# radhofan/Fairify

Hardware: AMD Instinct MI355X
Metric: % partitions verified + partitions/sec on AC suite at 1/2/4/8 MI355X (higher is better)
Workload: dtype fp32

## Files before the change

### fairify_amd/csrc/bindings.cpp

```cpp
#include <hip/hip_runtime.h>
#include <pybind11/pybind11.h>
#include <pybind11/stl.h>

#include <algorithm>
#include <cmath>
#include <cstring>
#include <cstdint>
#include <stdexcept>
#include <vector>

#include "kwargs.h"
#include "runtime_host.h"

extern "C" int fa_bounds_launch(const NetDesc& net, BoundArgs args, hipStream_t stream);
extern "C" int fa_crown_phase_launch(const NetDesc& net, CrownPhaseArgs a, hipStream_t stream);
extern "C" size_t fa_crown_phase_bytes(const NetDesc& net);
extern "C" int fa_point_try_launch(const NetDesc& net, BoundArgs a, hipStream_t stream);
extern "C" int fa_forward_launch(const NetDesc& net, FwdArgs a, hipStream_t stream);
extern "C" int fa_sim_launch(const NetDesc& net, SimArgs a, hipStream_t stream);
extern "C" int fa_sim_shaped(const NetDesc& net);
extern "C" int fa_sym_shaped(const NetDesc& net, unsigned long long fold_mask);
extern "C" int fa_crown_shaped(const NetDesc& net, int mask);
extern "C" int fa_refine_shaped(const NetDesc& net, int logit);
extern "C" int fa_rate_launch(const NetDesc& net, RateArgs a, hipStream_t stream);
extern "C" int fa_count_enum_launch(const NetDesc& net, EnumArgs a, hipStream_t stream);
extern "C" int fa_count_rows_launch(CountArgs a, hipStream_t stream);
extern "C" int fa_count_level_launch(CountArgs a, hipStream_t stream);
extern "C" int fa_ascent_launch(const NetDesc& net, AscentArgs a, hipStream_t stream);
extern "C" int fa_certify_launch(CertArgs a, hipStream_t stream);
extern "C" int fa_falsify_launch(const NetDesc& net, FalsifyArgs a, hipStream_t stream);
extern "C" int fa_prune_masks_launch(const NetDesc& net, int P, const int* counts, const float* ub, int ub_stride,
                                     const uint8_t* sym_dead, uint8_t* code, int* cnt, hipStream_t stream);
extern "C" int fa_heuristic_launch(const NetDesc& net, int Pu, const int64_t* rows, const float* lb, const float* ub,
                                   int stride, const uint8_t* code, double q50, double qlo, double qhi, uint8_t* hnew,
                                   uint8_t* hmerged, int* hcnt, hipStream_t stream);
extern "C" int fa_agree_launch(const NetDesc& net, const float* flat, int Pm, const int64_t* rows, const float* lo,
                               const float* hi, const int64_t* pids, const uint8_t* dead, int S, uint32_t seed,
                               int* agree, hipStream_t stream);

extern "C" int fa_decode_launch(const DecodeDesc& d, const int64_t* ids, int P, const float* chunk_lo,
                                const float* chunk_hi, float* lo, float* hi, hipStream_t stream);
extern "C" int fa_trace_marker_launch(int tag, int* sink, hipStream_t stream);
extern "C" int fa_beta_launch(const NetDesc& nd, BetaArgs a, hipStream_t stream);
extern "C" int fa_beta_config(const NetDesc& nd, int* wpb, int* wtl, size_t* bytes);
extern "C" int fa_beta_opt16_fits(const NetDesc& nd);
extern "C" size_t fa_beta_opt16_scratch_floats(const NetDesc& nd, int R);
extern "C" int fa_beta_opt16_launch(const NetDesc& nd, BetaArgs a, float* pgsum, float* pgn, hipStream_t stream);
extern "C" int fa_beta_level16_launch(const NetDesc& nd, BetaArgs a, hipStream_t stream);
extern "C" int fa_beta_opt16_feas_launch(const NetDesc& nd, BetaArgs a, hipStream_t stream);
extern "C" int fa_beta_feas16_launch(const NetDesc& nd, BetaArgs a, hipStream_t stream);
extern "C" int fa_knn_launch(const float* X, int n, int d, int k, int* idx, float* dist, hipStream_t stream);
extern "C" int fa_actdiff_launch(const NetDesc& net, const float* flat, const float* x, const float* xp, int npairs,
                                 float* sum_out, hipStream_t stream);
extern "C" int fa_pack_masks_launch(const uint8_t* src, int P, int N, int stride, int sel, uint8_t* out, int NB,
                                    unsigned long long* hash, hipStream_t stream);

template <typename T>
static T* P(uintptr_t p) { return reinterpret_cast<T*>(p); }

using fa_rt::gamma_up;

struct Net {
  NetDesc d;
  explicit Net(const std::vector<int>& dims, double unit) {
    if (dims.size() < 2 || dims.size() > FA_MAX_LAYERS + 1) throw std::invalid_argument("bad layer count");
    std::memset(&d, 0, sizeof(d));
    d.n_layers = (int)dims.size() - 1;
    int off = 0, noff = 0, mw = 0, mws = 0;
    for (size_t i = 0; i < dims.size(); ++i) {
      d.dims[i] = dims[i];
      mw = std::max(mw, dims[i]);
    }
    for (int l = 0; l < d.n_layers; ++l) {
      d.w_off[l] = off;
      off += dims[l] * dims[l + 1];
      d.b_off[l] = off;
      off += dims[l + 1];
      d.neuron_off[l] = noff;
      noff += dims[l + 1];
      mws = std::max(mws, dims[l] * dims[l + 1]);
      d.g_gemm[l] = gamma_up(2 * dims[l] + 1, unit);
      d.g_fwd[l] = gamma_up(dims[l] + 1, unit);
    }
    d.n_neurons = noff;
    d.n_hidden = noff - dims.back();
    d.max_width = mw;
    d.max_wsize = mws;
    d.unit = (float)unit;
    d.g_conc = gamma_up(dims[0] + 1, unit);
    d.g_one = gamma_up(1, unit);
    n_params = off;
    d.wperm_off = (off + 3) & ~3;
    int wp = 0;
    for (int l = 0; l < d.n_layers; ++l) wp += ((dims[l] + 15) / 16) * ((dims[l + 1] + 15) / 16) * 256;
    for (int l = 0; l < d.n_layers; ++l) wp += dims[l + 1];
    d.wperm_floats = (wp + 3) & ~3;
    total_floats = d.wperm_off + d.wperm_floats;
    d.pack_g = 1;
    if (d.n_layers >= 2 && dims[0] <= 16 && mw <= 16) {
      int mh = 0;
      for (int l = 1; l < d.n_layers; ++l) mh = std::max(mh, dims[l]);
      d.pack_g = mh <= 4 ? 4 : (mh <= 8 ? 2 : 1);
    }
    d.pack_off = total_floats;
    d.pack_floats = 0;
    if (d.pack_g > 1) {
      d.pack_floats = d.pack_g * 256 + (d.n_layers - 1) * 256 + d.n_layers * 16;
      total_floats += d.pack_floats;
    }
    d.wback_off = total_floats;
    int wb = 0;
    for (int l = 0; l < d.n_layers; ++l) wb += ((dims[l] + 15) / 16) * ((dims[l + 1] + 15) / 16) * 256;
    d.wback_floats = wb;
    total_floats += wb;
  }
  int n_params;
  int total_floats;
};

const NetDesc& fa_net_desc(py::handle h) { return h.cast<const Net&>().d; }
void register_bab(py::module& m);
void register_relu(py::module& m);
void register_beta(py::module& m);
extern "C" int fa_crown_launch(const NetDesc& net, BoundArgs a, hipStream_t stream);
extern "C" int fa_refine_launch(const NetDesc& net, BoundArgs a, hipStream_t stream);
extern "C" int fa_backward_launch(const NetDesc& net, BoundArgs a, hipStream_t stream);
extern "C" int fa_refine_crown_launch(const NetDesc& net, BoundArgs a, hipStream_t stream);
void register_csv(py::module& m);

using fa_rt::ckl;

static hipStream_t finish(Kw& k) {
  const hipStream_t s = reinterpret_cast<hipStream_t>(k.u64("stream"));
  k.done();
  return s;
}

static int dims(Kw& k, const char* key, int* idx, size_t cap, const char* too_many) {
  const std::vector<int> v = k.ints(key);
  if (v.size() > cap) throw std::invalid_argument(too_many);
  std::copy(v.begin(), v.end(), idx);
  return (int)v.size();
}

enum { OUT = 1, FORMS = 2, LAYERS = 4 };
template <typename A>
static A row_args(Kw& k, int req, const char* lo = "lo", const char* hi = "hi") {
  auto p = [&](const char* key, int group) { return (req & group) ? k.need<float>(key) : k.ptr<float>(key); };
  A a{};
  a.flat = k.need<const float>("flat");
  a.lo = k.need<const float>(lo);
  a.hi = k.need<const float>(hi);
  a.R = k.i("R");
  a.out_lb = p("out_lb", OUT);
  a.out_ub = p("out_ub", OUT);
  a.Lc = p("Lc", FORMS); a.L0 = p("L0", FORMS); a.Le = p("Le", FORMS);
  a.Uc = p("Uc", FORMS); a.U0 = p("U0", FORMS); a.Ue = p("Ue", FORMS);
  a.layer_lb = p("layer_lb", LAYERS);
  a.layer_ub = p("layer_ub", LAYERS);
  return a;
}
static BoundArgs bound_args(Kw& k, int req, const char* lo = "lo", const char* hi = "hi") {
  BoundArgs a = row_args<BoundArgs>(k, req, lo, hi);
  a.dead_in = k.ptr<const uint8_t>("dead_in");
  return a;
}

template <typename A>
static void fill_query(A& a, Kw& k, const char* too_many) {
  a.flat = k.need<const float>("flat");
  a.lo = k.need<const float>("lo");
  a.hi = k.need<const float>("hi");
  a.P = k.i("P");
  a.V = k.i("V");
  a.npa = dims(k, "pa", a.pa_idx, FA_MAX_PA, too_many);
  a.values = k.ptr<const int64_t>("values");
  a.Pp = k.i("Pp");
  a.pairs = k.ptr<const int64_t>("pairs");
}
template <typename A>
static void fill_samples(A& a, Kw& k, const char* too_many) {
  a.pids = k.need<const int64_t>("pids");
  a.n_samples = k.i("n_samples");
  a.seed = (uint32_t)k.u64("seed");
  a.nra = dims(k, "ra", a.ra_idx, FA_MAX_RA, too_many);
  a.tau = k.i("tau");
}
template <typename A>
static void fill_ascent(A& a, Kw& k, const char* too_many) {
  a.K = k.i("K");
  a.iters = k.i("iters");
  a.nfree = dims(k, "free", a.free_idx, 64, too_many);
  a.found = k.need<uint8_t>("found");
  a.wit_x = k.need<float>("wit_x");
  a.wit_xp = k.need<float>("wit_xp");
}

static BetaArgs beta_args(const Net& net, Kw& k) {
  BetaArgs a;
  std::memset(&a, 0, sizeof(a));
  a.flat = k.need<const float>("flat");
  a.wt = k.ptr<const float>("wt");
  a.R = k.i("R");
  a.npa = dims(k, "pa", a.pa_idx, FA_MAX_PA, "beta_level: too many PA dims");
  for (int q = 0; q < a.npa; ++q)
    if (a.pa_idx[q] < 0 || a.pa_idx[q] >= net.d.dims[0] || (q && a.pa_idx[q] <= a.pa_idx[q - 1]))
      throw std::invalid_argument("beta_level: PA dims must be increasing input indices");
  a.lo = k.need<const float>("lo");
  a.hi = k.need<const float>("hi");
  a.va = k.need<const float>("va");
  a.vb = k.need<const float>("vb");
  a.LBA = k.need<const float>("LBA");
  a.UBA = k.need<const float>("UBA");
  a.LBB = k.need<const float>("LBB");
  a.UBB = k.need<const float>("UBB");
  a.phA = k.need<const int8_t>("phA");
  a.phB = k.need<const int8_t>("phB");
  a.par = k.need<float>("par");
  a.t = k.need<float>("t");
  a.scratch = k.need<float>("scratch");
  a.iters = k.i("iters");
  a.lr_a = k.f("lr_a");
  a.lr_b = k.f("lr_b");
  a.lr_t = k.f("lr_t");
  a.decay = k.f("decay");
  a.lookahead = k.i("lookahead", 0);
  a.beta_pos = k.i("beta_pos", 1);
  const int flags = k.i("flags", 0);
  a.stall = flags & 1;
  a.pgap = (flags >> 1) & 3;
  a.feas = (flags >> 3) & 1;
  a.bound = k.ptr<double>("bound");
  a.split = k.ptr<int>("split");
  a.xstar = k.ptr<float>("xstar");
  a.binit = k.ptr<float>("binit");
  a.ramask = k.u64("ramask", 0);
  a.plo = k.ptr<const float>("plo");
  a.phi = k.ptr<const float>("phi");
  a.xpstar = k.ptr<float>("xpstar");
  a.gtie = k.ptr<float>("gtie");
  a.tau = k.f("tau", 0.f);
  a.osg = k.ptr<const int8_t>("osg");
  a.pgsum = k.ptr<const float>("pgsum");
  a.pgn = k.ptr<const float>("pgn");
  a.fpar = k.ptr<float>("fpar");
  a.fgt = k.ptr<float>("fgt");
  a.fval = k.ptr<double>("fval");
  if ((net.d.dims[0] < 64 && (a.ramask >> net.d.dims[0])) || (a.ramask && (!a.plo || !a.phi)))
    throw std::invalid_argument("beta_level: RA mask beyond the inputs or no x' box");
  return a;
}

PYBIND11_MODULE(_C, m) {
  m.doc() = "fairify_amd CDNA4 (gfx950) kernels";
  py::class_<Net>(m, "Net")
      .def(py::init<const std::vector<int>&, double>())
      .def_readonly("n_params", &Net::n_params)
      .def_readonly("total_floats", &Net::total_floats)
      .def_property_readonly("wperm_off", [](const Net& n) { return n.d.wperm_off; })
      .def_property_readonly("pack_g", [](const Net& n) { return n.d.pack_g; })
      .def_property_readonly("pack_off", [](const Net& n) { return n.d.pack_off; })
      .def_property_readonly("n_hidden", [](const Net& n) { return n.d.n_hidden; })
      .def_property_readonly("n_neurons", [](const Net& n) { return n.d.n_neurons; });

  m.def("bounds", [](const Net& net, py::kwargs kw) {
    Kw k("bounds", kw);
    const int symbolic = k.i("symbolic");
    BoundArgs a = bound_args(k, symbolic ? OUT | FORMS : OUT);
    a.symbolic = symbolic;
    a.G = k.i("G", 0);
    a.dead_out = k.ptr<uint8_t>("dead_out");
    a.fold = k.u64("fold", 0);
    a.phase_in = k.ptr<const int8_t>("phase_in");
    a.infeas = k.ptr<uint8_t>("infeas");
    ckl(fa_bounds_launch(net.d, a, finish(k)), "bounds");
  });

  m.def("crown_phase", [](const Net& net, py::kwargs kw) {
    Kw k("crown_phase", kw);
    CrownPhaseArgs a = row_args<CrownPhaseArgs>(k, OUT | FORMS | LAYERS);
    a.phase = k.ptr<const int8_t>("phase");
    a.infeas = k.ptr<const uint8_t>("infeas");
    a.split = k.need<int>("split");
    a.score = k.need<float>("score");
    a.low = k.ptr<float>("low");
    const int rc = fa_crown_phase_launch(net.d, a, finish(k));
    if (rc != 0) throw std::runtime_error("crown_phase launch failed, code " + std::to_string(rc));
  });

  m.def("relu_fits", [](const Net& net) { return fa_crown_phase_bytes(net.d) > 0; });

  m.def("crown", [](const Net& net, py::kwargs kw) {
    Kw k("crown", kw);
    const BoundArgs a = bound_args(k, OUT | FORMS | LAYERS);
    ckl(fa_crown_launch(net.d, a, finish(k)), "crown");
  });

  m.def("refine", [](const Net& net, py::kwargs kw) {
    Kw k("refine", kw);
    BoundArgs a = bound_args(k, LAYERS);
    a.phase_in = k.ptr<const int8_t>("phase_in");
    a.infeas = k.ptr<uint8_t>("infeas");
    const int rc = fa_refine_launch(net.d, a, finish(k));
    if (rc < -1) throw std::runtime_error("refine launch failed, code " + std::to_string(rc));
    return rc;
  });
  m.def("refine_crown", [](const Net& net, py::kwargs kw) {
    Kw k("refine_crown", kw);
    const BoundArgs a = bound_args(k, OUT | FORMS | LAYERS);
    const int rc = fa_refine_crown_launch(net.d, a, finish(k));
    if (rc < -1) throw std::runtime_error("refine_crown launch failed, code " + std::to_string(rc));
    return rc;
  });
  m.def("backward_bounds", [](const Net& net, py::kwargs kw) {
    Kw k("backward_bounds", kw);
    const BoundArgs a = bound_args(k, OUT | FORMS);
    const int rc = fa_backward_launch(net.d, a, finish(k));
    if (rc < -1) throw std::runtime_error("backward_bounds launch failed, code " + std::to_string(rc));
    return rc;
  });

  m.def("point_bounds", [](const Net& net, py::kwargs kw) {
    Kw k("point_bounds", kw);
    BoundArgs a = bound_args(k, OUT, "x", "x");
    a.row_open = k.ptr<const uint8_t>("row_open");
    a.open_mod = k.i("open_mod", 0);
    if (a.row_open && a.open_mod <= 0) throw std::invalid_argument("point_bounds: row_open needs open_mod > 0");
    const hipStream_t stream = finish(k);
    const int rc = fa_point_try_launch(net.d, a, stream);
    if (rc < 0) ckl(-rc, "point_bounds");
    if (rc == 0) ckl(fa_bounds_launch(net.d, a, stream), "point_bounds(ibp)");
  });

  m.def("forward", [](const Net& net, uintptr_t flat, uintptr_t x, int B, uintptr_t dead, uintptr_t out,
                      uintptr_t stream) {
    FwdArgs a{};
    a.flat = P<const float>(flat);
    a.x = P<const float>(x);
    a.B = B;
    a.dead = P<const uint8_t>(dead);
    a.out = P<float>(out);
    ckl(fa_forward_launch(net.d, a, (hipStream_t)stream), "forward");
  });

  m.def("sim", [](const Net& net, py::kwargs kw) {
    Kw k("sim", kw);
    SimArgs a{};
    fill_query(a, k, "too many PA/RA dims");
    fill_samples(a, k, "too many PA/RA dims");
    a.counts = k.need<int>("counts");
    a.found = k.need<uint8_t>("found");
    a.wit_x = k.need<float>("wit_x");
    a.wit_xp = k.need<float>("wit_xp");
    a.z0 = k.ptr<float>("z0");
    a.keys = k.ptr<int>("keys");
    a.split = k.i("split");
    a.regcount = k.i("regcount");
    if (a.split < 1 || (a.split > 1 && !a.keys)) throw std::invalid_argument("sim: split > 1 needs a keys buffer");
    ckl(fa_sim_launch(net.d, a, finish(k)), "sim");
  });
  m.def("sim_shaped", [](const Net& net) { return fa_sim_shaped(net.d) != 0; });
  m.def("sym_shaped", [](const Net& net, unsigned long long fold) { return fa_sym_shaped(net.d, fold) != 0; });
  m.def("crown_shaped", [](const Net& net, bool mask) { return fa_crown_shaped(net.d, mask) != 0; });
  m.def("refine_shaped", [](const Net& net, bool logit) { return fa_refine_shaped(net.d, logit) != 0; });

  m.def("rate", [](const Net& net, py::kwargs kw) {
    Kw k("rate", kw);
    RateArgs a{};
    fill_query(a, k, "too many PA/RA dims");
    fill_samples(a, k, "too many PA/RA dims");
    a.E = k.i("E");
    a.flips = k.need<int>("flips");
    a.amb = k.need<int>("amb");
    a.amb_idx = k.need<int>("amb_idx");
    a.split = k.i("split");
    const int rc = fa_rate_launch(net.d, a, finish(k));
    if (rc == -3) throw std::invalid_argument("rate: shape not covered (layer > 160, inputs > 32, V > 32 or E > 32)");
    ckl(rc, "rate");
  });

  m.def("count_enum", [](const Net& net, py::kwargs kw) {
    Kw k("count_enum", kw);
    EnumArgs a{};
    a.flat = k.need<const float>("flat");
    a.lo = k.need<const float>("lo");
    a.hi = k.need<const float>("hi");
    a.L = k.i("L");
    a.V = k.i("V");
    a.npa = dims(k, "pa", a.pa_idx, FA_MAX_PA, "too many PA/RA dims");
    a.values = k.need<const int64_t>("values");
    a.Pp = k.i("Pp");
    a.pairs = k.ptr<const int64_t>("pairs");
    a.nra = dims(k, "ra", a.ra_idx, FA_MAX_RA, "too many PA/RA dims");
    a.tau = k.i("tau");
    a.E = k.i("E");
    a.max_vol = k.i("max_vol");
    a.cert = k.need<int>("cert");
    a.amb = k.need<int>("amb");
    a.amb_idx = k.need<int>("amb_idx");
    a.blocks = k.i("blocks");
    if (a.Pp > 0 && !a.pairs) throw py::type_error("count_enum() missing required keyword argument 'pairs'");
    const int rc = fa_count_enum_launch(net.d, a, finish(k));
    if (rc == -3)
      throw std::invalid_argument(
          "count_enum: shape not covered (layer > 160, inputs > 32, V > 32, E > 32 or leaf volume > 65536)");
    ckl(rc, "count_enum");
  });
  auto count_args = [](Kw& k) {
    CountArgs a{};
    a.N = k.i("N");
    a.n0 = k.i("n0");
    a.V = k.i("V");
    a.npa = dims(k, "pa", a.pa_idx, FA_MAX_PA, "too many PA/RA dims");
    a.lo = k.need<const float>("lo");
    a.hi = k.need<const float>("hi");
    return a;
  };
  m.def("count_rows", [count_args](py::kwargs kw) {
    Kw k("count_rows", kw);
    CountArgs a = count_args(k);
    a.nra = dims(k, "ra", a.ra_idx, FA_MAX_RA, "too many PA/RA dims");
    a.tau = k.f("tau");
    a.values = k.need<const float>("values");
    a.rlo = k.need<float>("rlo");
    a.rhi = k.need<float>("rhi");
    a.plo = k.ptr<float>("plo");
    a.phi = k.ptr<float>("phi");
    ckl(fa_count_rows_launch(a, finish(k)), "count_rows");
  });
  m.def("count_level", [count_args](py::kwargs kw) {
    Kw k("count_level", kw);
    CountArgs a = count_args(k);
    a.part = k.need<const int>("part");
    a.lx = k.need<const float>("lx");
    a.ux = k.need<const float>("ux");
    a.lxp = k.need<const float>("lxp");
    a.uxp = k.need<const float>("uxp");
    a.Pp = k.i("Pp");
    a.pairs = k.ptr<const int64_t>("pairs");
    a.score = k.need<const float>("score");
    a.leaf_points = (long long)k.u64("leaf_points");
    a.code = k.need<uint8_t>("code");
    a.fair = k.need<long long>("fair");
    a.unfair = k.need<long long>("unfair");
    a.child_cnt = k.need<int>("child_cnt");
    a.olo = k.need<float>("olo");
    a.ohi = k.need<float>("ohi");
    a.opart = k.need<int>("opart");
    a.cap = k.i("cap");
    a.leaf_lo = k.need<float>("leaf_lo");
    a.leaf_hi = k.need<float>("leaf_hi");
    a.leaf_part = k.need<int>("leaf_part");
    a.leaf_cap = k.i("leaf_cap");
    a.counters = k.need<int>("counters");
    if (a.Pp > 0 && !a.pairs) throw py::type_error("count_level() missing required keyword argument 'pairs'");
    ckl(fa_count_level_launch(a, finish(k)), "count_level");
  });

  m.def("ascent", [](const Net& net, py::kwargs kw) {
    Kw k("ascent", kw);
    AscentArgs a{};
    fill_query(a, k, "too many PA/free dims");
    fill_ascent(a, k, "too many PA/free dims");
    a.x0 = k.need<const float>("x0");
    a.f0 = k.need<const float>("f0");
    a.q0 = k.need<const int>("q0");
    const int rc = fa_ascent_launch(net.d, a, finish(k));
    if (rc == -1) return false;
    ckl(rc, "ascent");
    return true;
  });

  m.def("falsify", [](const Net& net, py::kwargs kw) {
    Kw k("falsify", kw);
    FalsifyArgs a{};
    fill_query(a, k, "too many PA/RA/free dims");
    fill_samples(a, k, "too many PA/RA/free dims");
    fill_ascent(a, k, "too many PA/RA/free dims");
    if (a.tau <= 0) {
      a.nra = 0;
      std::fill_n(a.ra_idx, FA_MAX_RA, 0);
    }
    a.n_local = k.i("n_local");
    a.walk_k = k.i("walk_k");
    a.walk_steps = k.i("walk_steps");
    a.how = k.need<int8_t>("how");
    a.dseed = (uint32_t)k.u64("dseed");
    const int rc = fa_falsify_launch(net.d, a, finish(k));
    if (rc == 0) return false;
    if (rc < 0) ckl(-rc, "falsify");
    return true;
  });


  m.def("prune_masks", [](const Net& net, int Pn, uintptr_t counts, uintptr_t ub, int ub_stride, uintptr_t sym_dead,
                          uintptr_t code, uintptr_t cnt, uintptr_t stream) {
    ckl(fa_prune_masks_launch(net.d, Pn, P<const int>(counts), P<const float>(ub), ub_stride,
                                P<const uint8_t>(sym_dead), P<uint8_t>(code), P<int>(cnt), (hipStream_t)stream),
          "prune_masks");
  });

  m.def("heuristic", [](const Net& net, int Pu, uintptr_t rows, uintptr_t lb, uintptr_t ub, int stride, uintptr_t code,
                        double q50, double qlo, double qhi, uintptr_t hnew, uintptr_t hmerged, uintptr_t hcnt,
                        uintptr_t stream) {
    ckl(fa_heuristic_launch(net.d, Pu, P<const int64_t>(rows), P<const float>(lb), P<const float>(ub), stride,
                              P<const uint8_t>(code), q50, qlo, qhi, P<uint8_t>(hnew), P<uint8_t>(hmerged),
                              P<int>(hcnt), (hipStream_t)stream),
          "heuristic");
  });

  m.def("agree", [](const Net& net, uintptr_t flat, int Pm, uintptr_t rows, uintptr_t lo, uintptr_t hi, uintptr_t pids,
                    uintptr_t dead, int S, uint32_t seed, uintptr_t agree, uintptr_t stream) {
    const int rc = fa_agree_launch(net.d, P<const float>(flat), Pm, P<const int64_t>(rows), P<const float>(lo),
                                   P<const float>(hi), P<const int64_t>(pids), P<const uint8_t>(dead), S, seed,
                                   P<int>(agree), (hipStream_t)stream);
    if (rc == 0) return false;
    if (rc < 0) ckl(-rc, "agree");
    return true;
  });

  m.def("certify", [](py::kwargs kw) {
    Kw k("certify", kw);
    auto in = [&](const char* key) { return k.need<const float>(key); };
    CertArgs a{};
    a.Nn = k.i("Nn"); a.n0 = k.i("n0"); a.V = k.i("V"); a.Pp = k.i("Pp"); a.norient = k.i("norient");
    a.Lc = in("Lc"); a.L0 = in("L0"); a.Le = in("Le"); a.Uc = in("Uc"); a.U0 = in("U0"); a.Ue = in("Ue");
    a.olb = in("olb"); a.oub = in("oub");
    a.Lcp = in("Lcp"); a.L0p = in("L0p"); a.Lep = in("Lep"); a.Ucp = in("Ucp"); a.U0p = in("U0p"); a.Uep = in("Uep");
    a.olbp = in("olbp"); a.oubp = in("oubp");
    a.xlo = in("xlo"); a.xhi = in("xhi"); a.xplo = in("xplo"); a.xphi = in("xphi");
    a.pairs = k.ptr<const int64_t>("pairs");
    a.values = k.ptr<const int64_t>("values");
    a.npa = dims(k, "pa", a.pa_idx, FA_CMAX_PA, "too many PA/RA dims");
    a.nra = dims(k, "ra", a.ra_idx, FA_MAX_RA, "too many PA/RA dims");
    a.tau = k.f("tau");
    a.shared = k.need<const uint8_t>("shared");
    a.unit = k.f("unit");
    a.gmarg = std::nextafter(k.f("gmarg"), INFINITY);
    a.gmin = k.ptr<float>("gmin"); a.tstar = k.ptr<float>("tstar");
    a.open = k.need<uint8_t>("open"); a.score = k.need<float>("score"); a.split_dim = k.need<int64_t>("split_dim");
    a.cand_x = k.need<float>("cand_x"); a.cand_xp = k.need<float>("cand_xp");
    a.cand_v = k.need<int64_t>("cand_v"); a.cand_o = k.need<int64_t>("cand_o");
    a.scores = k.ptr<float>("scores"); a.leaf = k.ptr<uint8_t>("leaf");
    a.skip_closed = k.i("skip_closed", 0);
    a.status = k.ptr<const int8_t>("status"); a.part = k.ptr<const int>("part");
    a.smear = k.i("smear", 0);
    a.lay_lb = k.ptr<const float>("lay_lb"); a.lay_ub = k.ptr<const float>("lay_ub"); a.lay_N = k.i("lay_N", 0);
    a.W0T = k.ptr<const float>("W0T"); a.n1 = k.i("n1", 0);
    if ((a.status == nullptr) != (a.part == nullptr)) throw std::invalid_argument("certify: status and part go together");
    if (a.smear && (!a.lay_lb || !a.lay_ub || !a.W0T || a.n1 <= 0 || a.lay_N < a.n1))
      throw std::invalid_argument("certify: smear needs lay_lb, lay_ub, W0T and 0 < n1 <= lay_N");
    ckl(fa_certify_launch(a, finish(k)), "certify");
  });

  m.def("decode", [](std::vector<int> radix, std::vector<long long> div, std::vector<int> chunk_off,
                     std::vector<float> base_lo, std::vector<float> base_hi, uintptr_t ids, int Pn,
                     uintptr_t chunk_lo, uintptr_t chunk_hi, uintptr_t lo, uintptr_t hi, uintptr_t stream) {
    const size_t n0 = radix.size();
    if (n0 == 0 || n0 > FA_DECODE_MAX_DIMS || div.size() != n0 || chunk_off.size() != n0 || base_lo.size() != n0 ||
        base_hi.size() != n0)
      throw std::invalid_argument("decode: descriptor sizes");
    DecodeDesc d{};
    d.n0 = (int)n0;
    for (size_t k = 0; k < n0; ++k) {
      if (radix[k] < 0 || (radix[k] > 0 && div[k] <= 0)) throw std::invalid_argument("decode: radix/div");
      d.radix[k] = radix[k];
      d.div[k] = div[k];
      d.chunk_off[k] = chunk_off[k];
      d.base_lo[k] = base_lo[k];
      d.base_hi[k] = base_hi[k];
    }
    ckl(fa_decode_launch(d, P<const int64_t>(ids), Pn, P<const float>(chunk_lo), P<const float>(chunk_hi),
                           P<float>(lo), P<float>(hi), (hipStream_t)stream),
          "decode");
  });
  m.def("pack_masks", [](uintptr_t src, int Pn, int N, int stride, int sel, uintptr_t out, int NB, uintptr_t hash,
                         uintptr_t stream) {
    ckl(fa_pack_masks_launch(P<const uint8_t>(src), Pn, N, stride, sel, P<uint8_t>(out), NB,
                               P<unsigned long long>(hash), (hipStream_t)stream),
          "pack_masks");
  });
  m.def("knn", [](uintptr_t X, int n, int d, int k, uintptr_t idx, uintptr_t dist, uintptr_t stream) {
    ckl(fa_knn_launch(P<const float>(X), n, d, k, P<int>(idx), P<float>(dist), (hipStream_t)stream), "knn");
  });
  m.def("actdiff", [](const Net& net, uintptr_t flat, uintptr_t x, uintptr_t xp, int npairs, uintptr_t sum_out,
                      uintptr_t stream) {
    ckl(fa_actdiff_launch(net.d, P<const float>(flat), P<const float>(x), P<const float>(xp), npairs,
                            P<float>(sum_out), (hipStream_t)stream),
          "actdiff");
  });
  m.def("trace_marker", [](int tag, uintptr_t sink, uintptr_t stream) {
    ckl(fa_trace_marker_launch(tag, P<int>(sink), (hipStream_t)stream), "trace_marker");
  });
  m.def("beta_level", [](const Net& net, py::kwargs kw) {
    Kw k("beta_level", kw);
    const BetaArgs a = beta_args(net, k);
    return fa_beta_launch(net.d, a, finish(k));
  });
  m.def("beta_level16", [](const Net& net, py::kwargs kw) {
    Kw k("beta_level16", kw);
    const BetaArgs a = beta_args(net, k);
    return fa_beta_level16_launch(net.d, a, finish(k));
  });
  m.def("beta_opt16", [](const Net& net, py::kwargs kw) {
    Kw k("beta_opt16", kw);
    BetaArgs a = beta_args(net, k);
    float* pgsum = const_cast<float*>(a.pgsum);
    float* pgn = const_cast<float*>(a.pgn);
    a.wt = a.pgsum = a.pgn = nullptr;
    return fa_beta_opt16_launch(net.d, a, pgsum, pgn, finish(k));
  });
  m.def("beta_feas", [](const Net& net, py::kwargs kw) {
    Kw k("beta_feas", kw);
    BetaArgs a = beta_args(net, k);
    const int mode = k.i("mode");
    const hipStream_t st = finish(k);
    if (mode < 0 || mode > 3) throw std::invalid_argument("beta_feas: mode must be 0..3");
    if (mode != 0 && !a.fpar) throw std::invalid_argument("beta_feas: fpar required");
    a.lookahead = a.stall = a.pgap = 0;
    a.beta_pos = a.feas = 1;
    a.split = nullptr;
    a.xstar = a.binit = a.xpstar = nullptr;
    if (mode == 0) {
      a.fpar = a.fgt = nullptr;
      return fa_beta_launch(net.d, a, st);
    }
    if (mode == 1) return fa_beta_feas16_launch(net.d, a, st);
    if (mode == 2) return fa_beta_opt16_feas_launch(net.d, a, st);
    a.iters = 0;
    return fa_beta_launch(net.d, a, st);
  });
  m.def("beta_batched_fits", [](const Net& net) { return fa_beta_opt16_fits(net.d) != 0; });
  m.def("beta_opt16_scratch", [](const Net& net, int R) { return fa_beta_opt16_scratch_floats(net.d, R); });
  m.def("beta_config", [](const Net& net) {
    int w = 0, t = 0;
    size_t b = 0;
    const int rc = fa_beta_config(net.d, &w, &t, &b);
    return py::make_tuple(rc, w, t, b);
  });
  m.def("beta_fits", [](const Net& net) {
    int w = 0, t = 0;
    size_t b = 0;
    return fa_beta_config(net.d, &w, &t, &b) == 0;
  });
  m.def("arch", []() { return std::string("gfx950"); });
  m.def("prepare_lds", [] { return fa_lds_prepare(); });
  m.def("lds_registered", [] { return (int)fa_lds_registry().size(); });
  register_bab(m);
  register_relu(m);
  register_beta(m);
  m.def("mem_stats", [] {
    const fa_mem::Stats s = fa_mem::stats();
    py::dict d;
    d["dev_cached_bytes"] = s.dev_cached_bytes;
    d["dev_live_bytes"] = s.dev_live_bytes;
    d["host_cached_bytes"] = s.host_cached_bytes;
    d["host_live_bytes"] = s.host_live_bytes;
    d["dev_mallocs"] = s.dev_mallocs;
    d["dev_hits"] = s.dev_hits;
    d["host_mallocs"] = s.host_mallocs;
    d["host_hits"] = s.host_hits;
    d["driver_frees"] = s.driver_frees;
    return d;
  });
  m.def("mem_release_cached", [] { fa_mem::release_cached(); });
  register_csv(m);
}
```

### fairify_amd/csrc/symbolic.hip

```cpp
#include <hip/hip_runtime.h>

#include <tuple>

#include "args.h"
#include "launch.h"

#define FA_SYM_MAXC 48

struct SymCfg {
  int nc;
  int cdim[FA_SYM_MAXC];
  unsigned long long fold;
  int w_lds[FA_MAX_LAYERS];
  int b_lds[FA_MAX_LAYERS];
  int lds_floats;
  int stage_off;
  int stage_floats;
};

using SymShapeAny = FaShapeAny;
template <int... D>
using SymShape = FaShape<D...>;

struct SymBox {
  const BoundArgs* a;
  int node, v, n0;
  __device__ __forceinline__ float lo(int d) const {
    float x = a->lo[(size_t)node * n0 + d];
    if (a->V > 0)
      for (int k = 0; k < a->npa; ++k)
        if (a->pa_idx[k] == d) x = a->values[v * a->npa + k];
    return x;
  }
  __device__ __forceinline__ float hi(int d) const {
    float x = a->hi[(size_t)node * n0 + d];
    if (a->V > 0)
      for (int k = 0; k < a->npa; ++k)
        if (a->pa_idx[k] == d) x = a->values[v * a->npa + k];
    return x;
  }
};

__device__ __forceinline__ int fa_trot(int rho) { return rho >> 3; }

template <int NT, int PG = 1>
struct SymSlab {
  static constexpr int TS = 16 * NT + 4;
  static constexpr int TILE1 = 2 * 16 * TS;
  static constexpr int TILE = 2 * TILE1;
  static constexpr int BOX = 3 * FA_SYM_MAXC;
  static constexpr int BOXTAB = PG > 1 ? 2 * PG * 32 : 0;
  static constexpr int FLOATS = (TILE + 2 * PG * BOX + BOXTAB + 3) & ~3;
};

template <bool PAIR, int TM>
struct SymForm {
  static constexpr bool CR = !PAIR && TM >= 2;
};

__device__ __forceinline__ void fa_pq_to_ul(const f32x4& P, const f32x4& Q, int fc, float gg, f32x4& U,
                                            f32x4& L) {
  const float sl = (fc == 1 || fc == 3) ? 2.f * gg : 0.f;
#pragma unroll
  for (int i = 0; i < 4; ++i) {
    const float q = Q[i], e = sl * fabsf(q);
    U[i] = (P[i] + q) + e;
    L[i] = (P[i] - q) - e;
  }
}

template <int NT, bool PAIR, int PG = 1, bool CR = false, class S = SymShapeAny>
__device__ __forceinline__ bool fa_sym_epilogue(const NetDesc& net, const BoundArgs& a, const SymCfg& cfg,
                                                const float* smem, float* T, const float* bxv_in, const int* cdim_s,
                                                int l, int r_in, int node_in, int r2, int node2, bool v2, int lane,
                                                int jt0, const f32x4 (&U)[2][NT],
                                                const f32x4 (&Lq)[2][NT], float (&nu)[2][NT][4],
                                                float (&nlo)[2][NT][4]) {
  constexpr int TS = SymSlab<NT>::TS;
  constexpr bool CS = S::L > 0;
  const int col = lane & 15, grp = lane >> 4;
  const int n_out = CS ? S::dim(l + 1) : net.dims[l + 1];
  const float* sb = smem + cfg.b_lds[l];
  const bool last = CS ? l == S::L - 1 : l == net.n_layers - 1;
  const float gg = net.g_gemm[l];
  const float gc = net.g_conc;
  const float gi = net.g_one;
  const float unit = net.unit;
  const float gnext = last ? 0.f : (CR ? net.g_fwd[l + 1] : net.g_gemm[l + 1]);
  const int noff = net.neuron_off[l];
  const int nc = cfg.nc;
  const int n0 = CS ? S::dim(0) : net.dims[0];
  const int tsub = lane >> 5;
  const bool second = PAIR && tsub;
  constexpr int PS = 16 / PG;
  const int gbox = PG > 1 ? col / PS : 0;
  const int bidx = tsub * PG + gbox;
  const int r = PG > 1 ? r_in + bidx : (second ? r2 : r_in);
  const int node = PG > 1 ? (a.V > 0 ? r / a.V : r) : (second ? node2 : node_in);
  const float* bxv = bxv_in + (PG > 1 ? bidx : (second ? 1 : 0)) * SymSlab<NT, PG>::BOX;
  const int jt = PAIR ? jt0 : jt0 + tsub;
  const int n_out_t = n_out;
  const bool nl_act = PG > 1 ? r < a.R : (16 * jt < n_out_t && (!second || v2));
  const int ob = (lane >> 4) & 1;
  float* Trow = T + tsub * SymSlab<NT>::TILE1 + (ob * 16 + col) * TS + fa_trot(ob * 16 + col);
#pragma unroll
    for (int u = 0; u < 2; ++u)
#pragma unroll
      for (int ct = 0; ct < NT; ++ct)
#pragma unroll
        for (int i = 0; i < 4; ++i) {
          const int ru = 4 * grp + i, rl = 16 + 4 * grp + i;
          T[u * SymSlab<NT>::TILE1 + ru * TS + fa_trot(ru) + ct * 16 + col] = U[u][ct][i];
          T[u * SymSlab<NT>::TILE1 + rl * TS + fa_trot(rl) + ct * 16 + col] = Lq[u][ct][i];
        }
    __builtin_amdgcn_wave_barrier();
    const int j = PG > 1 ? col - gbox * PS : 16 * jt + col;
    const bool jv = j < n_out;
    float v[16 * NT];
#pragma unroll
    for (int c = 0; c < 16 * NT; ++c) v[c] = Trow[c];
    const float braw = sb[PG > 1 ? col : min(j, n_out - 1)];
    const float b = jv ? braw : 0.f;
    float s1 = 0.f, s2 = 0.f, mg = 0.f;
#pragma unroll
    for (int c = 4; c < 16 * NT; ++c) {
      const float av = fabsf(v[c]);
      s1 = fmaf(v[c], bxv[c], s1);
      s2 = fmaf(av, bxv[FA_SYM_MAXC + c], s2);
      mg = fmaf(av, bxv[2 * FA_SYM_MAXC + c], mg);
    }
    float mn = s1 - s2, mx = s1 + s2;
    const float cr = v[0];
    float er = v[1], ivr = v[2], ier = v[3];
    const float sgn = ob ? -1.f : 1.f;
    er *= sgn;
    ier *= sgn;
    const float c0 = cr + b;
    const float mgc = mg;
    mn += c0; mx += c0; mg += fabsf(c0);
    const float iv = ivr + b;
    const float eI = ier * (1.f + 2.f * gg) + gg * fabsf(b);
    const float e = er * (1.f + 2.f * gg) + gg * fabsf(b);
    float bound;
    if (ob == 0) bound = fminf(iv + gi * fabsf(iv) + eI, mx + gc * mg + e);
    else bound = fmaxf(iv - gi * fabsf(iv) - eI, mn - gc * mg - e);
    const float other = __shfl_xor(bound, 16, 64);
    const float ub = ob == 0 ? bound : other;
    const float lb = ob == 0 ? other : bound;
    if (nl_act && jv && a.layer_lb) {
      if (ob == 0) a.layer_ub[(size_t)r * net.n_neurons + noff + j] = ub;
      else a.layer_lb[(size_t)r * net.n_neurons + noff + j] = lb;
    }
    if (last) {
      if (nl_act && j == 0) {
        float* Cf = ob == 0 ? a.Uc : a.Lc;
        if (ob == 0) {
          a.out_ub[r] = ub; a.U0[r] = c0; a.Ue[r] = e;
        } else {
          a.out_lb[r] = lb; a.L0[r] = c0; a.Le[r] = e;
        }
        for (int d = 0; d < n0; ++d)
          if ((cfg.fold >> d) & 1ull) Cf[(size_t)r * n0 + d] = 0.f;
        for (int c = 0; c < nc; ++c) Cf[(size_t)r * n0 + cdim_s[c]] = Trow[4 + c];
      }
      return false;
    }
    bool forced = false, fact = false;
    if (nl_act && jv) {
      if (a.dead_in) forced = a.dead_in[(size_t)r * net.n_hidden + noff + j] != 0;
      else if (a.dead_part) forced = a.dead_part[(size_t)a.node_part[node] * net.n_hidden + noff + j] != 0;
      if (a.phase_in) {
        const int8_t ph = a.phase_in[(size_t)r * net.n_hidden + noff + j];
        forced = forced || ph < 0;
        fact = ph > 0;
        if (ob == 0 && a.infeas && ((ph < 0 && lb > 0.f) || (ph > 0 && ub < 0.f))) a.infeas[r] = 1;
      }
    }
    const bool isdead = ub <= 0.f;
    const bool isact = lb >= 0.f;
    if (nl_act && ob == 0 && jv && a.dead_out) a.dead_out[(size_t)r * net.n_hidden + noff + j] = isdead ? 1 : 0;
    const bool zero = isdead || forced || !jv;
    const float aa = mn - gc * mg + e;
    const float bb = mx + gc * mg + e;
    const bool chord = !zero && !isact && !fact && aa < 0.f;
    const float sc = (bb / (bb - aa)) * (1.f + 4.f * unit);
    const float shift = e - aa;
    const float cc = c0 * sc + sc * shift;
    const float sU = zero ? 0.f : (chord ? sc : 1.f);
    const float cU = zero ? 0.f : (chord ? cc : c0);
    const float mU = zero ? 0.f : (chord ? sc * mgc * (1.f + 8.f * unit) + fabsf(cc) : mg);
    const float eU = zero ? 0.f : (chord ? 4.f * unit * sc * (mg + fabsf(shift)) : e);
    const float aL = mn - gc * mg - e;
    const float bL = mx + gc * mg - e;
    const bool lam1 = !zero && (isact || ((bL > 0.f) && (bL > -aL)));
    const bool up = ob == 0;
    const float ivn = zero ? 0.f : fmaxf(up ? ub : lb, 0.f);
    const float s = up ? sU : (lam1 ? 1.f : 0.f);
    const float cnew = up ? cU : (lam1 ? c0 : 0.f);
    const float en = up ? eU : (lam1 ? e : 0.f);
    const float mgn = up ? mU : (lam1 ? mg : 0.f);
    const float mg_b = CR ? mgn + __shfl_xor(mgn, 16, 64) : mgn;
    const float iv_b = CR ? fmaxf(ivn, __shfl_xor(ivn, 16, 64)) : ivn;
    v[0] = cnew;
    v[1] = sgn * (en + gnext * mg_b);
    v[2] = ivn;
    v[3] = sgn * (gnext * iv_b);
#pragma unroll
    for (int c = 4; c < 16 * NT; ++c) v[c] *= s;
    if (nl_act) {
#pragma unroll
      for (int c = 0; c < 16 * NT; ++c) Trow[c] = v[c];
    }
    __builtin_amdgcn_wave_barrier();
#pragma unroll
    for (int u = 0; u < 2; ++u)
#pragma unroll
      for (int ct = 0; ct < NT; ++ct)
#pragma unroll
        for (int i = 0; i < 4; ++i) {
          const int ru = 4 * grp + i, rl = 16 + 4 * grp + i;
          const float xu = T[u * SymSlab<NT>::TILE1 + ru * TS + fa_trot(ru) + ct * 16 + col];
          const float xl = T[u * SymSlab<NT>::TILE1 + rl * TS + fa_trot(rl) + ct * 16 + col];
          nu[u][ct][i] = CR ? 0.5f * (xu + xl) : xu;
          nlo[u][ct][i] = CR ? 0.5f * (xu - xl) : xl;
        }
    __builtin_amdgcn_wave_barrier();
    return true;
}

template <int NT, int TM, bool PAIR, int PG = 1, class S = SymShapeAny>
__device__ __forceinline__ void fa_sym_layer(const NetDesc& net, const BoundArgs& a, const SymCfg& cfg,
                                             const float* smem, float* T, const float* bxv, const int* cdim_s,
                                             int l, int r, int node, int r2, int node2, bool v2, int lane,
                                             const float (&B)[NT][PAIR ? 2 : TM][2][4],
                                             float (&A)[NT][PAIR ? 2 : TM][2][4]) {
  constexpr int TMS = PAIR ? 2 : TM;
  constexpr bool CR = SymForm<PAIR, TM>::CR;
  constexpr int TS = SymSlab<NT>::TS;
  constexpr bool CS = S::L > 0;
  const int col = lane & 15, grp = lane >> 4;
  const int n_in = CS ? S::dim(l) : net.dims[l], n_out = CS ? S::dim(l + 1) : net.dims[l + 1];
  const int tin = (n_in + 15) >> 4, tout = (n_out + 15) >> 4;
  const float* sw = smem + cfg.w_lds[l];
  const float* sb = smem + cfg.b_lds[l];
  const bool last = CS ? l == S::L - 1 : l == net.n_layers - 1;
  const float gg = net.g_gemm[l];
  const float gc = net.g_conc;
  const float gi = net.g_one;
  const float unit = net.unit;
  const float gnext = last ? 0.f : net.g_gemm[l + 1];
  const int noff = net.neuron_off[l];
  const int nc = cfg.nc;
  const int n0 = CS ? S::dim(0) : net.dims[0];
  const bool nl_act = lane < 32;
  const int ob = (lane >> 4) & 1;
#ifndef FA_SYM_TIMING_NO_EPILOGUE
  if (PG > 1 && l == 0) {
    const float* boxtab = bxv + 2 * PG * SymSlab<NT, PG>::BOX;
    const float g0 = net.g_gemm[0];
    const int n0v = n0;
    f32x4 U[2][NT], Lq[2][NT];
#pragma unroll
    for (int u = 0; u < 2; ++u) {
#pragma unroll
      for (int ct = 0; ct < NT; ++ct) U[u][ct] = Lq[u][ct] = f32x4{0.f, 0.f, 0.f, 0.f};
#pragma unroll
      for (int g = 0; g < PG; ++g) {
        const float* bt = boxtab + (u * PG + g) * 32;
        const float4 w4 = reinterpret_cast<const float4*>(sw)[g * 64 + lane];
        const float wv[4] = {w4.x, w4.y, w4.z, w4.w};
#pragma unroll
        for (int i = 0; i < 4; ++i) {
          const int k = 4 * grp + i;
          const bool kv = k < n0v;
          const float xl = kv ? bt[k] : 0.f, xh = kv ? bt[16 + k] : 0.f;
          const bool folded = kv && ((cfg.fold >> k) & 1ull);
          const float m = fmaxf(fabsf(xl), fabsf(xh));
          const float wp = fmaxf(wv[i], 0.f), wn = fminf(wv[i], 0.f);
#pragma unroll
          for (int ct = 0; ct < NT; ++ct) {
            const int c = ct * 16 + col;
            float vu = 0.f, vl = 0.f;
            if (kv) {
              if (c >= 4) {
                vu = vl = (!folded && c - 4 < nc && cdim_s[c - 4] == k) ? 1.f : 0.f;
              } else if (c == 0) {
                vu = vl = folded ? xl : 0.f;
              } else if (c == 1) {
                vu = g0 * m; vl = -vu;
              } else if (c == 2) {
                vu = xh; vl = xl;
              } else {
                vu = g0 * fabsf(xh); vl = -(g0 * fabsf(xl));
              }
            }
            U[u][ct] = fa_mfma4(wp, vu, U[u][ct]);
            Lq[u][ct] = fa_mfma4(wp, vl, Lq[u][ct]);
            U[u][ct] = fa_mfma4(wn, vl, U[u][ct]);
            Lq[u][ct] = fa_mfma4(wn, vu, Lq[u][ct]);
          }
        }
      }
    }
    float nu[2][NT][4], nlo[2][NT][4];
    if (!fa_sym_epilogue<NT, PAIR, PG, CR, S>(net, a, cfg, smem, T, bxv, cdim_s, l, r, node, r2, node2, v2, lane, 0, U, Lq,
                                       nu, nlo))
      return;
#pragma unroll
    for (int u = 0; u < 2; ++u)
#pragma unroll
      for (int ct = 0; ct < NT; ++ct)
#pragma unroll
        for (int i = 0; i < 4; ++i) {
          A[ct][u][0][i] = nu[u][ct][i];
          A[ct][u][1][i] = nlo[u][ct][i];
        }
    return;
  }
  if (PG == 1 && last && n_out == 1) {
    constexpr int NB = PAIR ? 2 : 1;
    float su[NB][NT], sl[NB][NT];
#pragma unroll
    for (int bi = 0; bi < NB; ++bi)
#pragma unroll
      for (int ct = 0; ct < NT; ++ct) su[bi][ct] = sl[bi][ct] = 0.f;
#pragma unroll
    for (int t = 0; t < TM; ++t) {
      if (t >= tin) break;
      const float4 w4 = reinterpret_cast<const float4*>(sw)[t * 64 + grp * 16];
      const float wv[4] = {w4.x, w4.y, w4.z, w4.w};
#pragma unroll
      for (int i = 0; i < 4; ++i) {
        const float wp = fmaxf(wv[i], 0.f), wn = fminf(wv[i], 0.f);
#pragma unroll
        for (int bi = 0; bi < NB; ++bi)
#pragma unroll
          for (int ct = 0; ct < NT; ++ct) {
            const int bt = PAIR ? bi : t;
            if (CR) {
              su[bi][ct] = fmaf(wv[i], B[ct][bt][0][i], su[bi][ct]);
              sl[bi][ct] = fmaf(fabsf(wv[i]), B[ct][bt][1][i], sl[bi][ct]);
            } else {
              su[bi][ct] = fmaf(wp, B[ct][bt][0][i], fmaf(wn, B[ct][bt][1][i], su[bi][ct]));
              sl[bi][ct] = fmaf(wp, B[ct][bt][1][i], fmaf(wn, B[ct][bt][0][i], sl[bi][ct]));
            }
          }
      }
    }
    f32x4 U[2][NT], Lq[2][NT];
#pragma unroll
    for (int ct = 0; ct < NT; ++ct) U[1][ct] = Lq[1][ct] = f32x4{0.f, 0.f, 0.f, 0.f};
#pragma unroll
    for (int bi = 0; bi < NB; ++bi)
#pragma unroll
      for (int ct = 0; ct < NT; ++ct) {
        float xu = su[bi][ct], xl = sl[bi][ct];
        xu += __shfl_xor(xu, 16, 64);
        xl += __shfl_xor(xl, 16, 64);
        xu += __shfl_xor(xu, 32, 64);
        xl += __shfl_xor(xl, 32, 64);
        U[bi][ct] = f32x4{grp == 0 ? xu : 0.f, 0.f, 0.f, 0.f};
        Lq[bi][ct] = f32x4{grp == 0 ? xl : 0.f, 0.f, 0.f, 0.f};
        if (CR) fa_pq_to_ul(f32x4(U[bi][ct]), f32x4(Lq[bi][ct]), ct * 16 + col, gg, U[bi][ct], Lq[bi][ct]);
      }
    float nu[2][NT][4], nlo[2][NT][4];
    fa_sym_epilogue<NT, PAIR, PG, CR, S>(net, a, cfg, smem, T, bxv, cdim_s, l, r, node, r2, node2, v2, lane, 0, U, Lq,
                                  nu, nlo);
    return;
  }
#endif
#pragma unroll
  for (int jt0 = 0; jt0 < TM; jt0 += 2) {
    if (jt0 >= tout) break;
    f32x4 U[2][NT], Lq[2][NT];
#pragma unroll
    for (int u = 0; u < 2; ++u) {
      const int jt = jt0 + u;
#pragma unroll
      for (int ct = 0; ct < NT; ++ct) {
        U[u][ct] = f32x4{0.f, 0.f, 0.f, 0.f};
        Lq[u][ct] = f32x4{0.f, 0.f, 0.f, 0.f};
      }
      if (PAIR ? (jt0 > 0) : (jt >= tout || jt >= TM)) continue;
      const float4* wq = reinterpret_cast<const float4*>(sw) + (size_t)(PAIR ? 0 : jt) * tin * 64 + lane;
#pragma unroll
      for (int t = 0; t < TM; ++t) {
        if (t >= tin) break;
        const float4 w4 = wq[t * 64];
        const float wv[4] = {w4.x, w4.y, w4.z, w4.w};
#pragma unroll
        for (int i = 0; i < 4; ++i) {
          const float wp = fmaxf(wv[i], 0.f), wn = fminf(wv[i], 0.f);
#pragma unroll
          for (int ct = 0; ct < NT; ++ct) {
            const int bt = PAIR ? u : t;
            const float bu = B[ct][bt][0][i], bl = B[ct][bt][1][i];
            if (CR) {
              U[u][ct] = fa_mfma4(wv[i], bu, U[u][ct]);
              Lq[u][ct] = fa_mfma4(fabsf(wv[i]), bl, Lq[u][ct]);
            } else {
              U[u][ct] = fa_mfma4(wp, bu, U[u][ct]);
              Lq[u][ct] = fa_mfma4(wp, bl, Lq[u][ct]);
              U[u][ct] = fa_mfma4(wn, bl, U[u][ct]);
              Lq[u][ct] = fa_mfma4(wn, bu, Lq[u][ct]);
            }
          }
        }
      }
      if (CR) {
#pragma unroll
        for (int ct = 0; ct < NT; ++ct)
          fa_pq_to_ul(f32x4(U[u][ct]), f32x4(Lq[u][ct]), ct * 16 + col, gg, U[u][ct], Lq[u][ct]);
      }
    }
    float nu[2][NT][4], nlo[2][NT][4];
#ifdef FA_SYM_TIMING_NO_EPILOGUE
#pragma unroll
    for (int u = 0; u < 2; ++u)
#pragma unroll
      for (int ct = 0; ct < NT; ++ct)
#pragma unroll
        for (int i = 0; i < 4; ++i) {
          nu[u][ct][i] = U[u][ct][i] * 1e-3f;
          nlo[u][ct][i] = Lq[u][ct][i] * 1e-3f;
        }
    if (l == net.n_layers - 1) {
      if (lane == 0) a.out_lb[r] = nu[0][0][0] + nlo[0][0][1];
      continue;
    }
#else
    if (!fa_sym_epilogue<NT, PAIR, PG, CR, S>(net, a, cfg, smem, T, bxv, cdim_s, l, r, node, r2, node2, v2, lane, jt0, U,
                                       Lq, nu, nlo))
      continue;
#endif
#pragma unroll
    for (int u = 0; u < 2; ++u) {
      if (jt0 + u >= TMS) break;
#pragma unroll
      for (int ct = 0; ct < NT; ++ct)
#pragma unroll
        for (int i = 0; i < 4; ++i) {
          A[ct][jt0 + u][0][i] = nu[u][ct][i];
          A[ct][jt0 + u][1][i] = nlo[u][ct][i];
        }
    }
  }
}

#ifndef FA_SYM_WPE7
#define FA_SYM_WPE7 2
#endif
#ifndef FA_SYM_WPE4
#define FA_SYM_WPE4 2
#endif
#define FA_SYM_WAVES_PER_EU(NT, TM, PAIR) \
  ((PAIR) ? 3 : ((TM) == 2 ? 3 : ((TM) == 4 ? FA_SYM_WPE4 : ((TM) == 7 ? FA_SYM_WPE7 : 1))))

template <int NT, int TM, bool PAIR, int PG, class S, int... LS>
__device__ __forceinline__ void fa_sym_layers_c(std::integer_sequence<int, LS...>, const NetDesc& net,
                                                const BoundArgs& a, const SymCfg& cfg, const float* smem, float* T,
                                                const float* bxv, const int* cdim_s, int r, int node, int r2,
                                                int node2, bool v2, int lane, float (&XA)[NT][PAIR ? 2 : TM][2][4],
                                                float (&XB)[NT][PAIR ? 2 : TM][2][4]) {
  ((LS & 1 ? fa_sym_layer<NT, TM, PAIR, PG, S>(net, a, cfg, smem, T, bxv, cdim_s, LS, r, node, r2, node2, v2, lane,
                                               XB, XA)
           : fa_sym_layer<NT, TM, PAIR, PG, S>(net, a, cfg, smem, T, bxv, cdim_s, LS, r, node, r2, node2, v2, lane,
                                               XA, XB)),
   ...);
}

#ifndef FA_SYM_BIG_THREADS
#define FA_SYM_BIG_THREADS 512
#endif
#define FA_SYM_THREADS(TM) ((TM) == 7 ? FA_SYM_BIG_THREADS : FA_THREADS)

template <int NT, int TM, bool PAIR, int PG = 1, class S = SymShapeAny>
__global__ void __launch_bounds__(FA_SYM_THREADS(TM)) __attribute__((amdgpu_waves_per_eu(FA_SYM_WAVES_PER_EU(NT, TM, PAIR))))
fa_sym_kernel(NetDesc net, BoundArgs a, SymCfg cfg) {
  constexpr bool CR = SymForm<PAIR, TM>::CR;
  constexpr int TMS = PAIR ? 2 : TM;
  extern __shared__ __attribute__((aligned(16))) float smem[];
  const int tid = threadIdx.x;
  {
    const float4* src = reinterpret_cast<const float4*>(a.flat + cfg.stage_off);
    float4* dst = reinterpret_cast<float4*>(smem);
    for (int e = tid; e < (cfg.stage_floats >> 2); e += FA_SYM_THREADS(TM)) dst[e] = src[e];
  }
  int* cdim_s = reinterpret_cast<int*>(smem + cfg.lds_floats - FA_SYM_MAXC);
  for (int c = tid; c < FA_SYM_MAXC; c += FA_SYM_THREADS(TM)) cdim_s[c] = c < cfg.nc ? cfg.cdim[c] : -1;
  __syncthreads();
  const int lane = tid & 63;
  const int grp = lane >> 4;
  const int wave = tid >> 6;
  const int nw = FA_SYM_THREADS(TM) / 64;
  const int n0 = S::L > 0 ? S::dim(0) : net.dims[0];
  const int nc = cfg.nc;
  const float g0 = net.g_gemm[0];
  float* T = smem + cfg.lds_floats + wave * SymSlab<NT, PG>::FLOATS;
  float* bxv = T + SymSlab<NT>::TILE;
  const int tin0 = (n0 + 15) >> 4;
  int role[NT], cdm[NT];
#pragma unroll
  for (int ct = 0; ct < NT; ++ct) {
    const int c = ct * 16 + (lane & 15);
    role[ct] = c == 0 ? 1 : c == 1 ? 2 : c == 2 ? 3 : c == 3 ? 4 : (c - 4 < nc ? 0 : 5);
    cdm[ct] = (role[ct] == 0) ? cdim_s[c - 4] : -1;
  }
  constexpr int RPW = PAIR ? 2 * PG : 1;
  for (int r0 = (blockIdx.x * nw + wave) * RPW; r0 < a.R; r0 += gridDim.x * nw * RPW) {
    const int r = __builtin_amdgcn_readfirstlane(r0);
    const bool v2 = PAIR && r + 1 < a.R;
    const int rb = v2 ? r + 1 : r;
    if (a.skip_status) {
      bool any = false;
#pragma unroll
      for (int bi = 0; bi < RPW; ++bi) {
        const int rr = min(r + bi, a.R - 1);
        const int8_t s1 = a.skip_status[a.skip_part[a.V > 0 ? rr / a.V : rr]];
        any = any || s1 == 3 || s1 == 4;
      }
      if (!any) continue;
    }
    SymBox bxs[RPW];
#pragma unroll
    for (int bi = 0; bi < RPW; ++bi) {
      SymBox& bx = bxs[bi];
      const int rr = PG > 1 ? min(r + bi, a.R - 1) : (bi ? rb : r);
      bx.a = &a;
      bx.n0 = n0;
      bx.node = a.V > 0 ? rr / a.V : rr;
      bx.v = a.V > 0 ? rr - bx.node * a.V : 0;
      if (lane < FA_SYM_MAXC) {
        float* bv = bxv + bi * SymSlab<NT>::BOX;
        const int d = (lane >= 4 && lane - 4 < nc) ? cdim_s[lane - 4] : -1;
        const float l0 = d >= 0 ? bx.lo(d) : 0.f, h0 = d >= 0 ? bx.hi(d) : 0.f;
        float mid = 0.5f * (l0 + h0), rad = 0.5f * (h0 - l0), mm = fmaxf(fabsf(l0), fabsf(h0));
        const bool lattice = l0 == rintf(l0) && h0 == rintf(h0) && fabsf(l0) < 4194304.f && fabsf(h0) < 4194304.f;
        if (!lattice) {
          rad = nextafterf(fmaxf(h0 - mid, mid - l0), INFINITY);
          mm = nextafterf(fabsf(mid) + rad, INFINITY);
        }
        bv[lane] = mid;
        bv[FA_SYM_MAXC + lane] = rad;
        bv[2 * FA_SYM_MAXC + lane] = mm;
      }
      if (PG > 1 && lane < 32) {
        const int d = lane & 15;
        float* bt = bxv + 2 * PG * SymSlab<NT, PG>::BOX + bi * 32;
        bt[lane] = d < n0 ? (lane < 16 ? bx.lo(d) : bx.hi(d)) : 0.f;
      }
    }
    const SymBox& bx = bxs[0];
    float XA[NT][TMS][2][4], XB[NT][TMS][2][4];
#pragma unroll
    for (int t = 0; t < TMS; ++t) {
      if (PG > 1) break;
      if (!PAIR && t >= tin0) break;
      const SymBox& bt = bxs[PAIR ? t : 0];
#pragma unroll
      for (int i = 0; i < 4; ++i) {
        const int k = (PAIR ? 0 : 16 * t) + 4 * grp + i;
        float xl = 0.f, xh = 0.f;
        const bool kv = k < n0;
        if (kv) {
          xl = bt.lo(k);
          xh = bt.hi(k);
        }
        const bool folded = kv && ((cfg.fold >> k) & 1ull);
        const float m = fmaxf(fabsf(xl), fabsf(xh));
#pragma unroll
        for (int ct = 0; ct < NT; ++ct) {
          float vu = 0.f, vl = 0.f;
          if (kv) {
            switch (role[ct]) {
              case 0: vu = (!folded && cdm[ct] == k) ? 1.f : 0.f; vl = CR ? 0.f : vu; break;
              case 1: vu = folded ? xl : 0.f; vl = CR ? 0.f : vu; break;
              case 2: vu = CR ? 0.f : g0 * m; vl = CR ? g0 * m : -vu; break;
              case 3:
                vu = CR ? 0.5f * (xh + xl) : xh;
                vl = CR ? 0.5f * (xh - xl) : xl;
                break;
              case 4:
                vu = CR ? 0.5f * g0 * (fabsf(xh) - fabsf(xl)) : g0 * fabsf(xh);
                vl = CR ? 0.5f * g0 * (fabsf(xh) + fabsf(xl)) : -(g0 * fabsf(xl));
                break;
              default: break;
            }
          }
          XA[ct][t][0][i] = vu;
          XA[ct][t][1][i] = vl;
        }
      }
    }
    __builtin_amdgcn_wave_barrier();
    if constexpr (S::L > 0) {
      fa_sym_layers_c<NT, TM, PAIR, PG, S>(std::make_integer_sequence<int, S::L>{}, net, a, cfg, smem, T, bxv, cdim_s,
                                           r, bx.node, rb, bxs[RPW - 1].node, v2, lane, XA, XB);
    } else {
      for (int l = 0; l < net.n_layers; ++l) {
        if (l & 1)
          fa_sym_layer<NT, TM, PAIR, PG>(net, a, cfg, smem, T, bxv, cdim_s, l, r, bx.node, rb, bxs[RPW - 1].node, v2,
                                         lane, XB, XA);
        else
          fa_sym_layer<NT, TM, PAIR, PG>(net, a, cfg, smem, T, bxv, cdim_s, l, r, bx.node, rb, bxs[RPW - 1].node, v2,
                                         lane, XA, XB);
      }
    }
    __builtin_amdgcn_wave_barrier();
  }
}


namespace {

typedef void (*SymKernel)(NetDesc, BoundArgs, SymCfg);

template <int NT, int TM, bool PAIR = false, int PG = 1>
SymKernel sym_ptr() {
  return fa_sym_kernel<NT, TM, PAIR, PG>;
}

bool use_pack() {
  static const bool v = [] {
    const char* e = getenv("FAIRIFY_SYM_PACK");
    return !(e && *e == '0');
  }();
  return v;
}

SymKernel select_packed(int pg) {
  switch (pg) {
    case 2: return sym_ptr<1, 1, true, 2>();
    case 4: return sym_ptr<1, 1, true, 4>();
    default: return nullptr;
  }
}

bool use_pair() {
  static const bool v = [] {
    const char* e = getenv("FAIRIFY_SYM_PAIR");
    return !(e && *e == '0');
  }();
  return v;
}

int max_tm() {
  static const int v = [] {
    const char* e = getenv("FAIRIFY_SYM_MAX_TM");
    return (e && *e) ? atoi(e) : 10;
  }();
  return v;
}

#define FA_SYM_GRID(X) X(1, 1) X(1, 2) X(1, 4) X(1, 7) X(1, 10) X(2, 1) X(2, 2) X(2, 4) X(2, 10) X(3, 1) X(3, 2)

int tm_bucket(int NT, int TM) {
  if (TM > max_tm()) return 0;
  const int b = fa_tm_bucket(TM);
  if (NT == 2 && b == 7) return 10;
  if (NT == 3 && b > 2) return 0;
  return NT >= 1 && NT <= 3 ? b : 0;
}

SymKernel select_kernel(int NT, int tmb) {
  if (NT == 1 && tmb == 1 && use_pair()) return sym_ptr<1, 1, true>();
  switch (16 * NT + tmb) {
#define FA_SYM_CASE(NT_, TM_) \
  case 16 * NT_ + TM_: return sym_ptr<NT_, TM_>();
    FA_SYM_GRID(FA_SYM_CASE)
#undef FA_SYM_CASE
    default: return nullptr;
  }
}

#define FA_SYM_SHAPES(X)                                                                              \
  X(1, 4, false, 1, 13, 64, 32, 16, 8, 4, 1)                \
  X(2, 4, false, 1, 13, 64, 32, 16, 8, 4, 1)          \
  X(2, 4, false, 1, 16, 64, 32, 16, 8, 4, 1)                                                \
  X(1, 4, false, 1, 13, 64, 64, 1)                                                          \
  X(1, 4, false, 1, 13, 50, 1)                                                              \
  X(1, 7, false, 1, 13, 100, 100, 1)                                                        \
  X(1, 7, false, 1, 13, 100, 1)                                                             \
               \
  X(1, 1, true, 1, 13, 16, 8, 1)                                                            \
  X(1, 1, true, 1, 13, 12, 12, 1)                                                           \
  X(1, 1, true, 1, 13, 10, 10, 10, 10, 1)                                                  \
                                                         \
  X(1, 1, true, 2, 13, 5, 5, 1)                                                             \
  X(1, 1, true, 2, 13, 5, 5, 5, 5, 1)

constexpr int sym_key(int nt, int tm, bool pair, int pg) { return ((16 * nt + tm) * 2 + (pair ? 1 : 0)) * 8 + pg; }

struct SymPick {
  SymKernel k;
  int NT, tmb;
  bool pair;
  int pg;
  bool shaped;
};

SymPick pick_sym(const NetDesc& net, unsigned long long fold_mask, SymCfg& cfg) {
  SymPick p{};
  const int n0 = net.dims[0];
  if (n0 > 64) return p;
  cfg.fold = fold_mask;
  int nc = 0;
  for (int d = 0; d < n0; ++d)
    if (!((fold_mask >> d) & 1ull)) {
      if (nc >= FA_SYM_MAXC) return p;
      cfg.cdim[nc++] = d;
    }
  cfg.nc = nc;
  const int cols = nc + 4;
  p.NT = (cols + 15) / 16;
  p.tmb = tm_bucket(p.NT, fa_widest_tiles(net, 0, net.n_layers));
  SymKernel k = select_kernel(p.NT, p.tmb);
  if (!k) return p;
  p.pair = k == sym_ptr<1, 1, true>();
  p.pg = (p.pair && net.pack_g > 1 && net.dims[0] <= 16 && use_pack()) ? net.pack_g : 1;
  if (p.pg > 1) k = select_packed(p.pg);
  if (!k) return p;
  if (!fa_env_off("FAIRIFY_SYM_SHAPED")) {
#define FA_SYM_ENTRY(NT, TM, PAIR, PG, ...) \
  {sym_key(NT, TM, PAIR, PG), {__VA_ARGS__}, fa_sym_kernel<NT, TM, PAIR, PG, SymShape<__VA_ARGS__>>},
    static const std::vector<FaShaped<SymKernel>> v = {FA_SYM_SHAPES(FA_SYM_ENTRY)};
#undef FA_SYM_ENTRY
    if (const SymKernel ks = fa_find_shaped(v, net, sym_key(p.NT, p.tmb, p.pair, p.pg))) {
      k = ks;
      p.shaped = true;
    }
  }
  p.k = k;
  return p;
}

}

extern "C" int fa_sym_shaped(const NetDesc& net, unsigned long long fold_mask) {
  SymCfg cfg{};
  return pick_sym(net, fold_mask, cfg).shaped;
}

extern "C" int fa_sym_try_launch(const NetDesc& net, BoundArgs a, unsigned long long fold_mask,
                                 hipStream_t stream) {
  if (!a.symbolic || a.R <= 0) return 0;
  SymCfg cfg{};
  const SymPick p = pick_sym(net, fold_mask, cfg);
  const SymKernel k = p.k;
  if (!k) return 0;
  const int NT = p.NT, tmb = p.tmb, pg = p.pg;
  const bool pair0 = p.pair;
  int off = 0;
  if (pg > 1) {
    cfg.w_lds[0] = 0;
    off = pg * 256;
    for (int l = 1; l < net.n_layers; ++l) {
      cfg.w_lds[l] = off;
      off += 256;
    }
    for (int l = 0; l < net.n_layers; ++l) {
      cfg.b_lds[l] = off;
      off += 16;
    }
    if (off != net.pack_floats) return -1;
    cfg.stage_off = net.pack_off;
  } else {
    off = fa_lay_weights(net, net.n_layers, cfg.w_lds, 0);
    off = fa_lay_biases(net, net.n_layers, cfg.b_lds, off);
    off = ((off + 3) & ~3);
    if (off != net.wperm_floats) return -1;
    cfg.stage_off = net.wperm_off;
  }
  cfg.stage_floats = off;
  off += FA_SYM_MAXC;
  cfg.lds_floats = off;
  int slab = 0;
  switch (NT) {
    case 1:
      slab = pg == 2 ? SymSlab<1, 2>::FLOATS : pg == 4 ? SymSlab<1, 4>::FLOATS : SymSlab<1>::FLOATS;
      break;
    case 2: slab = SymSlab<2>::FLOATS; break;
    default: slab = SymSlab<3>::FLOATS; break;
  }
  const int threads = (!pair0 && NT == 1 && tmb == 7) ? FA_SYM_BIG_THREADS : FA_THREADS;
  const int rows_per_block = (threads / 64) * (pair0 ? 2 * pg : 1);
  const size_t bytes = (size_t)(off + (threads / 64) * slab) * sizeof(float);
  if (bytes > 160 * 1024) return 0;
  const int per_cu = fa_blocks_per_cu((const void*)k, threads, bytes);
  if (!per_cu) return -4;
  long long blocks = (a.R + rows_per_block - 1) / rows_per_block;
  const long long cap = (long long)fa_device_cus() * per_cu;
  if (blocks > cap) blocks = cap;
  hipLaunchKernelGGL(k, dim3((unsigned)blocks), dim3(threads), bytes, stream, net, a, cfg);
  const hipError_t e = hipGetLastError();
  return e == hipSuccess ? 1 : -(int)e;
}

#define FA_SYM_LDS(NT, TM) FA_LDS_K((sym_ptr<NT, TM>())),
#define FA_SYM_SHAPE_LDS(NT, TM, PAIR, PG, ...) FA_LDS_K((fa_sym_kernel<NT, TM, PAIR, PG, SymShape<__VA_ARGS__>>)),
FA_LDS_REGISTER(FA_SYM_GRID(FA_SYM_LDS) FA_LDS_K((sym_ptr<1, 1, true>())), FA_LDS_K((sym_ptr<1, 1, true, 2>())),
                FA_LDS_K((sym_ptr<1, 1, true, 4>())));
FA_LDS_REGISTER(FA_SYM_SHAPES(FA_SYM_SHAPE_LDS));
#undef FA_SYM_LDS
#undef FA_SYM_SHAPE_LDS
```

### fairify_amd/ops/hip.py

```python
from __future__ import annotations

import os
import threading
from typing import Optional, Sequence

import torch

from . import ext
from . import reference as ref


def _stream(dev) -> int:
    return torch.cuda.current_stream(dev).cuda_stream


_LAZY_LOCK = threading.Lock()


def _net(be):
    n = getattr(be, "_hipnet", None)
    if n is None:
        with _LAZY_LOCK:
            n = getattr(be, "_hipnet", None)
            if n is None:
                dims = [be.mlp.n_in] + be.mlp.widths
                n = ext().Net(dims, be.unit)
                assert n.total_floats == be.flat.numel(), (n.total_floats, be.flat.numel())
                be._hipnet = n
    return n


def _c(t: torch.Tensor, dtype, shape=None, name="tensor") -> torch.Tensor:
    if t.dtype != dtype:
        t = t.to(dtype)
    t = t.contiguous()
    if shape is not None and tuple(t.shape) != tuple(shape):
        raise ValueError(f"{name}: expected shape {tuple(shape)}, got {tuple(t.shape)}")
    return t


def _fold_mask(fold: Sequence[int], n0: int) -> int:
    m = 0
    for d in fold:
        if not 0 <= int(d) < min(n0, 64):
            raise ValueError(f"fold dim {d} out of range")
        m |= 1 << int(d)
    return m


def _ptr(t: Optional[torch.Tensor]) -> int:
    return 0 if t is None else t.data_ptr()


def _ptrs(**tensors) -> dict:
    return {k: t.data_ptr() for k, t in tensors.items() if t is not None}


def _bound_kw(be, lo, hi, dead=None, res=None, layer_lb=None, layer_ub=None):
    R, n0 = lo.shape
    t = dict(flat=be.flat, lo=_c(lo, torch.float32, (R, n0), "lo"), hi=_c(hi, torch.float32, (R, n0), "hi"),
             dead_in=None if dead is None else _c(dead, torch.uint8, (R, be.n_hidden), "dead"),
             layer_lb=layer_lb, layer_ub=layer_ub)
    if res is not None:
        t.update(out_lb=res.out_lb, out_ub=res.out_ub, Lc=res.Lc, L0=res.L0, Le=res.Le, Uc=res.Uc, U0=res.U0,
                 Ue=res.Ue)
    return dict(_ptrs(**t), R=R, stream=_stream(lo.device)), t


def _layer_views(be, lay_lb, lay_ub):
    offs = [0]
    for w in be.mlp.widths:
        offs.append(offs[-1] + w)
    n = len(be.mlp.widths)
    return [lay_lb[:, offs[i]:offs[i + 1]] for i in range(n)], [lay_ub[:, offs[i]:offs[i + 1]] for i in range(n)]


def decode(grid, ids: torch.Tensor):
    dev = ids.device
    ids = _c(ids, torch.int64, (ids.shape[0],), "ids")
    tabs = grid.__dict__.setdefault("_dev_decode", {})
    key = str(dev)
    if key not in tabs:
        with _LAZY_LOCK:
            if key not in tabs:
                d = grid.decode_desc()
                cl = torch.from_numpy(d["chunk_lo"]).to(dev) if d["chunk_lo"].size else torch.zeros(1, device=dev)
                ch = torch.from_numpy(d["chunk_hi"]).to(dev) if d["chunk_hi"].size else torch.zeros(1, device=dev)
                torch.cuda.current_stream(dev).synchronize()
                tabs[key] = (d, cl, ch)
    d, cl, ch = tabs[key]
    n0 = int(d["radix"].shape[0])
    Pn = int(ids.shape[0])
    lo = torch.empty(Pn, n0, dtype=torch.float32, device=dev)
    hi = torch.empty(Pn, n0, dtype=torch.float32, device=dev)
    if Pn:
        ext().decode(d["radix"].tolist(), d["div"].tolist(), d["chunk_off"].tolist(), d["base_lo"].tolist(),
                     d["base_hi"].tolist(), ids.data_ptr(), Pn, cl.data_ptr(), ch.data_ptr(), lo.data_ptr(),
                     hi.data_ptr(), _stream(dev))
    return lo, hi


def pack_masks(masks: torch.Tensor, sel: int = 0xFF):
    m = _c(masks, torch.uint8, name="masks")
    if m.dim() != 2:
        raise ValueError("masks: expected [P, N]")
    Pn, N = m.shape
    NB = (N + 7) // 8
    out = torch.empty(Pn, NB, dtype=torch.uint8, device=m.device)
    hsh = torch.empty(Pn, dtype=torch.int64, device=m.device)
    if Pn and N:
        ext().pack_masks(m.data_ptr(), Pn, N, N, int(sel), out.data_ptr(), NB, hsh.data_ptr(), _stream(m.device))
    return out, hsh


KNN_K = (1, 2, 3, 4, 5, 6, 7, 8, 10, 16)


def knn(X: torch.Tensor, k: int):
    X = _c(X, torch.float32, name="X")
    n, d = X.shape
    if not 1 <= d <= 64 or k not in KNN_K or k > n:
        raise ValueError(f"knn: unsupported shape n={n} d={d} k={k}")
    idx = torch.empty(n, k, dtype=torch.int32, device=X.device)
    dist = torch.empty(n, k, dtype=torch.float32, device=X.device)
    ext().knn(X.data_ptr(), n, d, k, idx.data_ptr(), dist.data_ptr(), _stream(X.device))
    return idx, dist


def activation_delta_sum(be, x: torch.Tensor, xp: torch.Tensor) -> torch.Tensor:
    P_ = x.shape[0]
    x = _c(x, torch.float32, (P_, be.n0), "x")
    xp = _c(xp, torch.float32, (P_, be.n0), "xp")
    out = torch.zeros(be.mlp.n_neurons, dtype=torch.float32, device=x.device)
    if P_:
        ext().actdiff(_net(be), be.flat.data_ptr(), x.data_ptr(), xp.data_ptr(), P_, out.data_ptr(),
                      _stream(x.device))
    return out


def trace_marker(dev, tag: int) -> None:
    ext().trace_marker(int(tag), 0, _stream(dev))


def forward(be, x: torch.Tensor, dead: Optional[torch.Tensor] = None) -> torch.Tensor:
    shp = x.shape[:-1]
    x2 = _c(x.reshape(-1, be.n0), torch.float32, name="x")
    B = x2.shape[0]
    out = torch.empty(B, dtype=torch.float32, device=x.device)
    if B == 0:
        return out.view(shp)
    d = None
    if dead is not None:
        d = _c(dead.reshape(-1, be.n_hidden), torch.uint8, (B, be.n_hidden), "dead")
    ext().forward(_net(be), be.flat.data_ptr(), x2.data_ptr(), B, _ptr(d), out.data_ptr(), _stream(x.device))
    return out.view(shp)


def activation_counts(be, x: torch.Tensor) -> torch.Tensor:
    return ref.activation_counts(be.ws, be.bs, x)


def point_bounds(be, x: torch.Tensor, dead: Optional[torch.Tensor] = None):
    R = x.shape[0]
    x2 = _c(x, torch.float32, (R, be.n0), "x")
    lb = torch.empty(R, dtype=torch.float32, device=x.device)
    ub = torch.empty(R, dtype=torch.float32, device=x.device)
    d = None
    if dead is not None:
        d = _c(dead, torch.uint8, (R, be.n_hidden), "dead")
    if R:
        ext().point_bounds(_net(be), **_ptrs(flat=be.flat, x=x2, dead_in=d, out_lb=lb, out_ub=ub), R=R,
                           stream=_stream(x.device))
    return lb, ub


def bounds(be, lo: torch.Tensor, hi: torch.Tensor, mode: str = "symbolic", dead: Optional[torch.Tensor] = None,
           keep_layers: bool = False, G: int = 0, fold: Sequence[int] = (),
           phase: Optional[torch.Tensor] = None) -> ref.BoundResult:
    R, n0 = lo.shape
    if n0 != be.n0:
        raise ValueError(f"box width {n0} != network input {be.n0}")
    dev = lo.device
    sym = 1 if mode == "symbolic" else 0
    f32 = dict(dtype=torch.float32, device=dev)
    res = ref.BoundResult(out_lb=torch.empty(R, **f32), out_ub=torch.empty(R, **f32))
    if sym:
        res.Lc = torch.empty(R, n0, **f32)
        res.L0 = torch.empty(R, **f32)
        res.Le = torch.empty(R, **f32)
        res.Uc = torch.empty(R, n0, **f32)
        res.U0 = torch.empty(R, **f32)
        res.Ue = torch.empty(R, **f32)
    N = be.mlp.n_neurons
    lay_lb = lay_ub = None
    if keep_layers:
        lay_lb = torch.empty(R, N, **f32)
        lay_ub = torch.empty(R, N, **f32)
    dead_out = torch.empty(R, be.n_hidden, dtype=torch.uint8, device=dev) if be.n_hidden else None
    ph = infeas = None
    if phase is not None:
        ph = _c(phase, torch.int8, (R, be.n_hidden), "phase")
        infeas = torch.zeros(R, dtype=torch.uint8, device=dev)
    kw, _keep = _bound_kw(be, lo, hi, dead, res, lay_lb, lay_ub)
    if R:
        ext().bounds(_net(be), **kw, **_ptrs(dead_out=dead_out, phase_in=ph, infeas=infeas), symbolic=sym, G=G,
                     fold=_fold_mask(fold, n0))
    if infeas is not None:
        res.infeasible = infeas.bool()
    if keep_layers:
        res.layer_lb, res.layer_ub = _layer_views(be, lay_lb, lay_ub)
        res.lay_lb_full, res.lay_ub_full = lay_lb, lay_ub
    if dead_out is not None:
        res.dead_u8 = dead_out
        res.dead = dead_out.view(torch.bool)
    return res


def crown(be, lo: torch.Tensor, hi: torch.Tensor, res: ref.BoundResult, dead: Optional[torch.Tensor] = None):
    R, n0 = lo.shape
    N = be.mlp.n_neurons
    if res.Lc is None or res.layer_lb is None:
        raise ValueError("crown needs symbolic bounds with keep_layers=True")
    lay_lb = torch.cat(res.layer_lb, dim=1).contiguous() if isinstance(res.layer_lb, list) else res.layer_lb
    lay_ub = torch.cat(res.layer_ub, dim=1).contiguous() if isinstance(res.layer_ub, list) else res.layer_ub
    if lay_lb.shape[1] != N:
        pad = torch.zeros(R, N - lay_lb.shape[1], dtype=torch.float32, device=lo.device)
        lay_lb = torch.cat([lay_lb, pad], dim=1).contiguous()
        lay_ub = torch.cat([lay_ub, pad], dim=1).contiguous()
    kw, _keep = _bound_kw(be, lo, hi, dead, res, lay_lb, lay_ub)
    if R:
        ext().crown(_net(be), **kw)
    return res


def refine(be, lo: torch.Tensor, hi: torch.Tensor, res: ref.BoundResult, dead: Optional[torch.Tensor] = None,
           phase: Optional[torch.Tensor] = None):
    R, n0 = lo.shape
    if res.lay_lb_full is None:
        raise ValueError("refine needs symbolic bounds with keep_layers=True (HIP layout)")
    kw, _keep = _bound_kw(be, lo, hi, dead, None, res.lay_lb_full, res.lay_ub_full)
    ph = _c(phase, torch.int8, (R, be.n_hidden), "phase") if phase is not None else None
    infeas = torch.zeros(R, dtype=torch.uint8, device=lo.device) if phase is not None else None
    if R:
        ext().refine(_net(be), **kw, **_ptrs(phase_in=ph, infeas=infeas))
    if infeas is not None:
        res.infeasible = infeas.bool() if res.infeasible is None else (res.infeasible | infeas.bool())
    Nh = be.n_hidden
    if Nh:
        res.dead = res.lay_ub_full[:, :Nh] <= 0
        res.dead_u8 = res.dead.to(torch.uint8)
        res.active = res.lay_lb_full[:, :Nh] >= 0
    return res


def backward_bounds(be, lo: torch.Tensor, hi: torch.Tensor, dead: Optional[torch.Tensor] = None,
                    keep_layers: bool = True) -> Optional[ref.BoundResult]:
    R, n0 = lo.shape
    f32 = dict(dtype=torch.float32, device=lo.device)
    res = ref.BoundResult(out_lb=torch.empty(R, **f32), out_ub=torch.empty(R, **f32),
                          Lc=torch.empty(R, n0, **f32), L0=torch.empty(R, **f32), Le=torch.empty(R, **f32),
                          Uc=torch.empty(R, n0, **f32), U0=torch.empty(R, **f32), Ue=torch.empty(R, **f32))
    N = be.mlp.n_neurons
    lay_lb = torch.empty(R, N, **f32) if keep_layers else None
    lay_ub = torch.empty(R, N, **f32) if keep_layers else None
    kw, keep = _bound_kw(be, lo, hi, dead, res, lay_lb, lay_ub)
    if R and ext().backward_bounds(_net(be), **kw) == -1:
        return None
    if keep_layers:
        res.layer_lb, res.layer_ub = _layer_views(be, lay_lb, lay_ub)
        res.lay_lb_full, res.lay_ub_full = lay_lb, lay_ub
        Nh = be.n_hidden
        res.dead = lay_ub[:, :Nh] <= 0
        d = keep["dead_in"]
        if d is not None:
            res.dead = res.dead | d.bool()
        res.active = (lay_lb[:, :Nh] >= 0) & ~res.dead
    return res


def crown_phase(be, lo: torch.Tensor, hi: torch.Tensor, res: ref.BoundResult, phase: Optional[torch.Tensor] = None):
    R, n0 = lo.shape
    dev = lo.device
    if res.lay_lb_full is None:
        raise ValueError("crown_phase needs bounds(..., keep_layers=True) from the HIP path")
    kw, _keep = _bound_kw(be, lo, hi, None, res, res.lay_lb_full, res.lay_ub_full)
    ph = _c(phase, torch.int8, (R, be.n_hidden), "phase") if phase is not None else None
    split = torch.full((R, 2), -1, dtype=torch.int32, device=dev)
    score = torch.zeros(R, 2, dtype=torch.float32, device=dev)
    low = torch.zeros(R, 2, dtype=torch.float32, device=dev)
    infeas = res.infeasible.to(torch.uint8).contiguous() if res.infeasible is not None else None
    if R:
        ext().crown_phase(_net(be), **kw, **_ptrs(phase=ph, infeas=infeas, split=split, score=score, low=low))
    return ref.PhaseCrown(low=low, split=split.long(), score=score), None


def smear_w0t(W0: torch.Tensor) -> torch.Tensor:
    n0, n1 = W0.shape
    if n0 > 32:
        raise ValueError("smear scores need n0 <= 32")
    out = torch.zeros(n1, 16 if n0 <= 16 else 32, dtype=torch.float32, device=W0.device)
    out[:, :n0] = W0.to(torch.float32).abs().T
    return out


def pair_certify(be, res_x, res_xp, xlo, xhi, xplo, xphi, pairs, values, pa, shared, relaxed, *, ra=(), tau=0.0,
                 skip_closed=False, status=None, part=None, smear=False, lay_lb=None, lay_ub=None, W0T=None,
                 prefill=None, full=False):
    Nn, n0 = xlo.shape
    dev = xlo.device
    V = values.shape[0]
    Pp = pairs.shape[0]
    norient = 2 if relaxed else 1
    ra = [int(i) for i in ra]
    if any(not 0 <= i < n0 for i in ra):
        raise ValueError("ra dim out of range")
    extra = {}
    if (status is None) != (part is None):
        raise ValueError("status and part go together")
    if status is not None:
        status = _c(status, torch.int8, None, "status")
        part = _c(part, torch.int32, (Nn,), "part")
        if status.dim() != 1 or (Nn and not 0 <= int(part.min()) <= int(part.max()) < status.shape[0]):
            raise ValueError("part indexes status [P]")
        extra.update(_ptrs(status=status, part=part))
    if skip_closed:
        extra["skip_closed"] = 1
    if smear:
        if lay_lb is None or lay_ub is None or W0T is None or lay_lb.dim() != 2:
            raise ValueError("smear needs lay_lb, lay_ub and W0T")
        lay_N, n1 = lay_lb.shape[1], W0T.shape[0]
        lay_lb = _c(lay_lb, torch.float32, (Nn * V, lay_N), "lay_lb")
        lay_ub = _c(lay_ub, torch.float32, (Nn * V, lay_N), "lay_ub")
        W0T = _c(W0T, torch.float32, (n1, 16 if n0 <= 16 else 32), "W0T")
        if not 0 < n1 <= lay_N:
            raise ValueError("smear: the first layer's n1 neurons lead the lay_N layer bounds")
        extra.update(_ptrs(lay_lb=lay_lb, lay_ub=lay_ub, W0T=W0T), smear=1, lay_N=lay_N, n1=n1)
    xlo = _c(xlo, torch.float32, (Nn, n0), "xlo")
    xhi = _c(xhi, torch.float32, (Nn, n0), "xhi")
    xplo = _c(xplo, torch.float32, (Nn, n0), "xplo")
    xphi = _c(xphi, torch.float32, (Nn, n0), "xphi")
    for r in (res_x, res_xp):
        if r.Lc is None or tuple(r.Lc.shape) != (Nn * V, n0):
            raise ValueError("pair_certify needs symbolic forms for Nn*V rows")
    pairs_c = _c(pairs, torch.int64, (Pp, 2), "pairs")
    values_c = _c(values, torch.int64, None, "values")
    sh = _c(shared, torch.uint8, (n0,), "shared")
    Q = Pp * norient

    def new(*shape, dtype=torch.float32):
        t = torch.empty(*shape, dtype=dtype, device=dev)
        return t if prefill is None else t.fill_(prefill)

    gmin = new(Nn, Q)
    tstar = new(Nn, Q)
    open_ = new(Nn, dtype=torch.uint8)
    score = new(Nn)
    split = new(Nn, dtype=torch.int64)
    cx = new(Nn, n0)
    cxp = new(Nn, n0)
    cv = new(Nn, dtype=torch.int64)
    co = new(Nn, dtype=torch.int64)
    forms = {}
    for r, p in ((res_x, ""), (res_xp, "p")):
        for key, t in (("Lc", r.Lc), ("L0", r.L0), ("Le", r.Le), ("Uc", r.Uc), ("U0", r.U0), ("Ue", r.Ue),
                       ("olb", r.out_lb), ("oub", r.out_ub)):
            forms[key + p] = _c(t, torch.float32)
    scores = new(Nn, 2 * n0)
    leaf = new(Nn, dtype=torch.uint8)
    if Nn:
        pa_l = [int(i) for i in pa.tolist()]
        if any(not 0 <= i < n0 for i in pa_l) or tuple(values_c.shape) != (V, len(pa_l)):
            raise ValueError("pa dims out of range or values not [V, npa]")
        ext().certify(Nn=Nn, n0=n0, V=V, Pp=Pp, norient=norient, pa=pa_l, ra=ra,
                      tau=float(tau), unit=be.unit, gmarg=ref.gamma(2 * n0 + 4, be.unit), stream=_stream(dev), **extra,
                      **_ptrs(xlo=xlo, xhi=xhi, xplo=xplo, xphi=xphi, pairs=pairs_c, values=values_c, shared=sh,
                              gmin=gmin, tstar=tstar, open=open_, score=score, split_dim=split, cand_x=cx,
                              cand_xp=cxp, cand_v=cv, cand_o=co, scores=scores, leaf=leaf, **forms))
    dec = ref.PairDecision(open_=open_.bool(), score=score, split_dim=split, cand_x=cx, cand_xp=cxp,
                           cand_v=cv, cand_orient=co)
    if full:
        return dec, dict(gmin=gmin, tstar=tstar, scores=scores, leaf=leaf, open_u8=open_)
    return dec


def _parse_sim_blocks(v: Optional[str]) -> int:
    if v is None or v.strip() == "":
        return 0
    try:
        n = int(v)
    except ValueError:
        raise ValueError(f"FAIRIFY_SIM_BLOCKS={v!r}: expected a non-negative integer") from None
    if n < 0:
        raise ValueError(f"FAIRIFY_SIM_BLOCKS={v!r}: expected a non-negative integer")
    return n


_SIM_BLOCKS = _parse_sim_blocks(os.environ.get("FAIRIFY_SIM_BLOCKS"))
_SIM_BLOCKS_ENV: Optional[str] = None


def _sim_split(P: int, n_samples: int) -> int:
    target = _SIM_BLOCKS if _SIM_BLOCKS_ENV is None else _parse_sim_blocks(os.environ.get("FAIRIFY_SIM_BLOCKS"))
    if not P or target <= P:
        return 1
    tiles = (n_samples + 63) // 64
    return max(1, min(tiles, -(-target // P)))


_SIM_REGCOUNT = os.environ.get("FAIRIFY_SIM_REGCOUNT", "1").strip() != "0"
_SIM_REGCOUNT_ENV: Optional[str] = None


def _sim_regcount() -> bool:
    if _SIM_REGCOUNT_ENV is None:
        return _SIM_REGCOUNT
    return os.environ.get("FAIRIFY_SIM_REGCOUNT", "1").strip() != "0"


def _query_kw(be, q, lo, hi, pids, values, pairs):
    P, n0 = lo.shape
    Pp = pairs.shape[0]
    t = dict(flat=be.flat, lo=_c(lo, torch.float32, (P, n0), "lo"), hi=_c(hi, torch.float32, (P, n0), "hi"),
             values=_c(values, torch.int64, None, "values"), pairs=_c(pairs, torch.int64, (Pp, 2), "pairs"))
    kw = dict(P=P, V=int(values.shape[0]), pa=list(q.pa_idx), Pp=int(Pp), stream=_stream(lo.device))
    if pids is not None:
        t["pids"] = _c(pids, torch.int64, (P,), "pids")
        kw.update(ra=list(q.ra_idx) if q.relaxed else [], tau=int(q.tau) if q.relaxed else 0)
    kw.update(_ptrs(**t))
    return kw, t


def simulate(be, q, lo, hi, pids, n_samples, seed, values, pairs, bisect_pairs, bisect_steps, return_z0=False):
    from ..engine.sim import SimResult, boundary_walk

    P, n0 = lo.shape
    dev = lo.device
    kw, t = _query_kw(be, q, lo, hi, pids, values, pairs)
    split = _sim_split(P, n_samples)
    counts = (torch.zeros if split > 1 else torch.empty)(P, be.mlp.n_neurons, dtype=torch.int32, device=dev)
    keys = torch.full((P,), 0x7FFFFFFF, dtype=torch.int32, device=dev) if split > 1 else None
    found = torch.zeros(P, dtype=torch.uint8, device=dev)
    wx = torch.zeros(P, n0, dtype=torch.float32, device=dev)
    wxp = torch.zeros(P, n0, dtype=torch.float32, device=dev)
    walk = bool(bisect_pairs and bisect_steps)
    z0 = torch.empty(P, n_samples, dtype=torch.float32, device=dev) if (walk or return_z0) else None
    if P and n_samples:
        kw["tau"] = int(q.tau)
        ext().sim(_net(be), **kw, **_ptrs(counts=counts, found=found, wit_x=wx, wit_xp=wxp, z0=z0, keys=keys),
                  n_samples=n_samples, seed=int(seed) & 0xFFFFFFFF, split=split, regcount=int(_sim_regcount()))
    res = SimResult(counts=counts, found=found.bool(), wit_x=wx, wit_xp=wxp)
    if return_z0:
        res.z0 = z0
    if walk:
        boundary_walk(be, q, t["lo"], t["hi"], t["pids"], n_samples, seed, t["values"], t["pairs"], res, z0,
                      bisect_pairs, bisect_steps)
    return res


_RATE_BLOCKS = 1024
_RATE_EMPTY = 0x7FFFFFFF


def rate_split_max(n_samples: int) -> int:
    return max(1, (n_samples + 63) // 64)


def _rate_split(P: int, n_samples: int) -> int:
    if not P or P >= _RATE_BLOCKS:
        return 1
    return max(1, min(rate_split_max(n_samples), _RATE_BLOCKS // P))


def rate_counts(be, q, lo, hi, pids, n_samples, seed, values, pairs, split: Optional[int] = None):
    from .rate import AMB_SLOTS, MAX_OFFSETS, offset_vectors

    P, n0 = lo.shape
    dev = lo.device
    if n0 != be.n0:
        raise ValueError(f"lo: expected [P, {be.n0}], got {tuple(lo.shape)}")
    npa = len(q.pa_idx)
    if values.dim() != 2 or values.shape[1] != npa:
        raise ValueError(f"values: expected [V, {npa}], got {tuple(values.shape)}")
    V = int(values.shape[0])
    Pp = int(pairs.shape[0])
    kw, t = _query_kw(be, q, lo, hi, pids, values, pairs)
    pairs_c = t["pairs"]
    if not 1 <= V <= 32:
        raise ValueError(f"rate: {V} PA assignments, the kernel covers 1..32")
    if Pp and (int(pairs_c.min()) < 0 or int(pairs_c.max()) >= V):
        raise ValueError("pairs: index outside [0, V)")
    E = int(offset_vectors(q).shape[0])
    assert E <= MAX_OFFSETS
    n_samples = int(n_samples)
    if n_samples < 0 or n_samples >= _RATE_EMPTY:
        raise ValueError(f"rate: bad sample count {n_samples}")
    if max([be.n0] + list(be.widths)) > 160 or be.n0 > 32:
        raise ValueError("rate: the kernel covers layers up to 160 wide and up to 32 inputs")
    if split is None:
        split = _rate_split(P, n_samples)
    if not 1 <= int(split) <= rate_split_max(n_samples):
        raise ValueError(f"rate: split {split} outside 1..{rate_split_max(n_samples)}")
    flips = torch.zeros(P, dtype=torch.int32, device=dev)
    amb = torch.zeros(P, dtype=torch.int32, device=dev)
    idx = torch.full((P, AMB_SLOTS), _RATE_EMPTY, dtype=torch.int32, device=dev)
    if P and n_samples:
        ext().rate(_net(be), **kw, **_ptrs(flips=flips, amb=amb, amb_idx=idx), n_samples=n_samples,
                   seed=int(seed) & 0xFFFFFFFF, E=E, split=int(split))
        idx = idx.masked_fill((amb > AMB_SLOTS)[:, None], _RATE_EMPTY).sort(dim=1).values
    return flips, amb, idx


_ENUM_BLOCKS = 1024
_ENUM_POINTS = 1024


def _count_shape(be, q, values, pairs, what):
    from .rate import offset_vectors

    npa = len(q.pa_idx)
    if values.dim() != 2 or values.shape[1] != npa:
        raise ValueError(f"values: expected [V, {npa}], got {tuple(values.shape)}")
    V, Pp = int(values.shape[0]), int(pairs.shape[0])
    if not 1 <= V <= 32:
        raise ValueError(f"{what}: {V} PA assignments, the kernels cover 1..32")
    if Pp and (int(pairs.min()) < 0 or int(pairs.max()) >= V):
        raise ValueError("pairs: index outside [0, V)")
    E = int(offset_vectors(q).shape[0])
    return V, Pp, E


def count_enum(be, q, lo, hi, values, pairs, max_vol: Optional[int] = None, blocks: Optional[int] = None):
    from .count import MAX_LEAF_POINTS, free_dims, volumes
    from .rate import AMB_SLOTS

    L, n0 = lo.shape
    dev = lo.device
    if n0 != be.n0:
        raise ValueError(f"lo: expected [L, {be.n0}], got {tuple(lo.shape)}")
    lo = _c(lo, torch.float32, (L, n0), "lo")
    hi = _c(hi, torch.float32, (L, n0), "hi")
    values = _c(values, torch.int64, None, "values")
    pairs = _c(pairs, torch.int64, (pairs.shape[0], 2), "pairs")
    V, Pp, E = _count_shape(be, q, values, pairs, "count_enum")
    if max([be.n0] + list(be.widths)) > 160 or be.n0 > 32:
        raise ValueError("count_enum: the kernel covers layers up to 160 wide and up to 32 inputs")
    if max_vol is None:
        max_vol = int(volumes(lo, hi, free_dims(q)).max()) if L else 1
    if not 1 <= int(max_vol) <= MAX_LEAF_POINTS:
        raise ValueError(f"count_enum: leaf volume {max_vol} outside 1..{MAX_LEAF_POINTS}")
    if blocks is None:
        blocks = min(max(L, 1), max(_ENUM_BLOCKS, L * int(max_vol) // _ENUM_POINTS))
    if L and not 1 <= int(blocks) <= L:
        raise ValueError(f"count_enum: {blocks} workgroups outside 1..{L}")
    cert = torch.zeros(L, dtype=torch.int32, device=dev)
    amb = torch.zeros(L, dtype=torch.int32, device=dev)
    idx = torch.full((L, AMB_SLOTS), _RATE_EMPTY, dtype=torch.int32, device=dev)
    if L:
        ext().count_enum(_net(be), **_ptrs(flat=be.flat, lo=lo, hi=hi, values=values, pairs=pairs if Pp else None,
                                           cert=cert, amb=amb, amb_idx=idx),
                         L=L, V=V, pa=list(q.pa_idx), Pp=Pp, ra=list(q.ra_idx) if q.relaxed else [],
                         tau=int(q.tau) if q.relaxed else 0, E=E, max_vol=int(max_vol), blocks=int(blocks),
                         stream=_stream(dev))
        idx = idx.masked_fill((amb > AMB_SLOTS)[:, None], _RATE_EMPTY).sort(dim=1).values
    return cert, amb, idx


def count_rows(be, q, lo, hi, values):
    N, n0 = lo.shape
    dev = lo.device
    lo = _c(lo, torch.float32, (N, n0), "lo")
    hi = _c(hi, torch.float32, (N, n0), "hi")
    npa = len(q.pa_idx)
    values = _c(values, torch.float32, None, "values")
    if values.dim() != 2 or values.shape[1] != npa or values.shape[0] < 1:
        raise ValueError(f"values: expected [V, {npa}], got {tuple(values.shape)}")
    if any(not 0 <= d < n0 for d in list(q.pa_idx) + list(q.ra_idx)):
        raise ValueError("count_rows: PA / RA dim outside the inputs")
    V = int(values.shape[0])
    f32 = dict(dtype=torch.float32, device=dev)
    rlo, rhi = torch.empty(N * V, n0, **f32), torch.empty(N * V, n0, **f32)
    plo = phi = None
    if q.relaxed:
        plo, phi = torch.empty(N * V, n0, **f32), torch.empty(N * V, n0, **f32)
    if N:
        ext().count_rows(**_ptrs(lo=lo, hi=hi, values=values, rlo=rlo, rhi=rhi, plo=plo, phi=phi), N=N, n0=n0, V=V,
                         pa=list(q.pa_idx), ra=list(q.ra_idx) if q.relaxed else [],
                         tau=float(q.tau) if q.relaxed else 0.0, stream=_stream(dev))
    return (rlo, rhi, plo, phi) if q.relaxed else (rlo, rhi, rlo, rhi)


def count_level(be, q, lo, hi, part, lx, ux, lxp, uxp, pairs, score, leaf_points, fair, unfair, child_cnt,
                part_checked: bool = False):
    N, n0 = lo.shape
    dev = lo.device
    lo = _c(lo, torch.float32, (N, n0), "lo")
    hi = _c(hi, torch.float32, (N, n0), "hi")
    part = _c(part, torch.int32, (N,), "part")
    V = lx.numel() // max(N, 1)
    t = {k: _c(v, torch.float32, (N * V,), k) for k, v in dict(lx=lx.reshape(-1), ux=ux.reshape(-1),
                                                                lxp=lxp.reshape(-1), uxp=uxp.reshape(-1)).items()}
    pairs = _c(pairs, torch.int64, (pairs.shape[0], 2), "pairs")
    Pp = int(pairs.shape[0])
    score = _c(score.to(dev), torch.float32, (n0,), "score")
    P = fair.shape[0]
    for name, x, dt in (("fair", fair, torch.int64), ("unfair", unfair, torch.int64), ("child_cnt", child_cnt, torch.int32)):
        if x.dtype != dt or tuple(x.shape) != (P,) or not x.is_contiguous() or x.device != dev:
            raise ValueError(f"{name}: expected a contiguous [{P}] {dt} tensor on {dev}")
    if N and not part_checked and (int(part.min()) < 0 or int(part.max()) >= P):
        raise ValueError("part: partition index outside [0, P)")
    if N and V < 1:
        raise ValueError("count_level: no rows")
    if any(not 0 <= d < n0 for d in q.pa_idx):
        raise ValueError("count_level: PA dim outside the inputs")
    if not 1 <= int(leaf_points) < 2 ** 62:
        raise ValueError(f"count_level: bad leaf size {leaf_points}")
    f32 = dict(dtype=torch.float32, device=dev)
    i32 = dict(dtype=torch.int32, device=dev)
    code = torch.empty(N, dtype=torch.uint8, device=dev)
    clo, chi, cpart = torch.empty(2 * N, n0, **f32), torch.empty(2 * N, n0, **f32), torch.empty(2 * N, **i32)
    llo, lhi, lpart = torch.empty(N, n0, **f32), torch.empty(N, n0, **f32), torch.empty(N, **i32)
    counters = torch.zeros(3, **i32)
    if N:
        ext().count_level(**_ptrs(lo=lo, hi=hi, part=part, pairs=pairs if Pp else None, score=score, code=code,
                                  fair=fair, unfair=unfair, child_cnt=child_cnt, olo=clo, ohi=chi, opart=cpart,
                                  leaf_lo=llo, leaf_hi=lhi, leaf_part=lpart, counters=counters, **t),
                          N=N, n0=n0, V=V, pa=list(q.pa_idx), Pp=Pp, leaf_points=int(leaf_points), cap=2 * N,
                          leaf_cap=N, stream=_stream(dev))
    return code, (clo, chi, cpart), (llo, lhi, lpart), counters


def ascent(be, q, lo, hi, x0, f0, q0, iters, values, pairs, free_dims):
    P, K, n0 = x0.shape
    dev = x0.device
    if tuple(lo.shape) != (P, n0):
        raise ValueError(f"lo: expected shape {(P, n0)}, got {tuple(lo.shape)}")
    kw, _keep = _query_kw(be, q, lo, hi, None, values, pairs)
    x0_c = _c(x0, torch.float32, (P, K, n0), "x0")
    f0_c = _c(f0, torch.float32, (P, K), "f0")
    q0_c = _c(q0, torch.int32, (P, K), "q0")
    found = torch.zeros(P, dtype=torch.uint8, device=dev)
    wx = torch.zeros(P, n0, dtype=torch.float32, device=dev)
    wxp = torch.zeros(P, n0, dtype=torch.float32, device=dev)
    if P == 0:
        return found.bool(), wx, wxp
    ok = ext().ascent(_net(be), **kw, **_ptrs(x0=x0_c, f0=f0_c, q0=q0_c, found=found, wit_x=wx, wit_xp=wxp), K=K,
                      iters=int(iters), free=[int(d) for d in free_dims])
    if not ok:
        return None
    return found.bool(), wx, wxp


def falsify(be, q, lo, hi, pids, values, pairs, seed, n_samples, n_local, walk_k, walk_steps, k_starts, iters,
            free_dims, dseed: int = 0):
    P, n0 = lo.shape
    dev = lo.device
    Pp = pairs.shape[0]
    kw, t = _query_kw(be, q, lo, hi, pids, values, pairs)
    if t["values"].numel() != kw["V"] * len(q.pa_idx):
        raise ValueError("values: expected [V, n_pa]")
    found = torch.zeros(P, dtype=torch.uint8, device=dev)
    wx = torch.zeros(P, n0, dtype=torch.float32, device=dev)
    wxp = torch.zeros(P, n0, dtype=torch.float32, device=dev)
    how = torch.zeros(P, dtype=torch.int8, device=dev)
    if P == 0 or Pp == 0 or n_samples <= 0:
        return found.bool(), wx, wxp, how
    ok = ext().falsify(_net(be), **kw, **_ptrs(found=found, wit_x=wx, wit_xp=wxp, how=how), n_samples=int(n_samples),
                       n_local=int(n_local), seed=int(seed) & 0xFFFFFFFF, walk_k=int(walk_k),
                       walk_steps=int(walk_steps), K=int(k_starts), iters=int(iters),
                       free=[int(d) for d in free_dims], dseed=int(dseed) & 0xFFFFFFFF)
    if not ok:
        return None
    return found.bool(), wx, wxp, how


def prune_masks(be, counts: torch.Tensor, lay_ub: torch.Tensor, sym_dead: Optional[torch.Tensor]):
    P, N = counts.shape
    dev = counts.device
    counts_c = _c(counts, torch.int32, (P, be.mlp.n_neurons), "counts")
    ub_c = _c(lay_ub, torch.float32, (P, N), "lay_ub")
    sd = None
    if sym_dead is not None:
        sd = _c(sym_dead, torch.uint8, (P, be.n_hidden), "sym_dead")
    code = torch.empty(P, N, dtype=torch.uint8, device=dev)
    cnt = torch.empty(P, 3, dtype=torch.int32, device=dev)
    if P:
        ext().prune_masks(_net(be), P, counts_c.data_ptr(), ub_c.data_ptr(), N, _ptr(sd), code.data_ptr(),
                          cnt.data_ptr(), _stream(dev))
    return code, cnt


PM_CAND, PM_B, PM_S, PM_ST, PM_SCAND = 1, 2, 4, 8, 16


def heuristic(be, rows: torch.Tensor, lay_lb: torch.Tensor, lay_ub: torch.Tensor, code: torch.Tensor, perc: float):
    Pu = rows.shape[0]
    P, N = lay_ub.shape
    dev = lay_ub.device
    rows_c = _c(rows, torch.int64, (Pu,), "rows")
    lb_c = _c(lay_lb, torch.float32, (P, N), "lay_lb")
    ub_c = _c(lay_ub, torch.float32, (P, N), "lay_ub")
    code_c = _c(code, torch.uint8, (P, N), "code")
    hnew = torch.empty(Pu, N, dtype=torch.uint8, device=dev)
    hmerged = torch.empty(Pu, N, dtype=torch.uint8, device=dev)
    cnt = torch.empty(Pu, 2, dtype=torch.int32, device=dev)
    if Pu:
        ext().heuristic(_net(be), Pu, rows_c.data_ptr(), lb_c.data_ptr(), ub_c.data_ptr(), N, code_c.data_ptr(),
                        50.0 / 100.0, float(perc) / 100.0, (100.0 - float(perc)) / 100.0, hnew.data_ptr(),
                        hmerged.data_ptr(), cnt.data_ptr(), _stream(dev))
    return hnew, hmerged, cnt


def agree(be, rows: torch.Tensor, lo: torch.Tensor, hi: torch.Tensor, pids: torch.Tensor, dead: torch.Tensor,
          n_samples: int, seed: int):
    Pm = rows.shape[0]
    P, n0 = lo.shape
    dev = lo.device
    rows_c = _c(rows, torch.int64, (Pm,), "rows")
    lo_c = _c(lo, torch.float32, (P, n0), "lo")
    hi_c = _c(hi, torch.float32, (P, n0), "hi")
    pids_c = _c(pids, torch.int64, (P,), "pids")
    dead_c = _c(dead, torch.uint8, (Pm, be.n_hidden), "dead")
    out = torch.zeros(Pm, 3, dtype=torch.int32, device=dev)
    if Pm == 0:
        return out
    ok = ext().agree(_net(be), be.flat.data_ptr(), Pm, rows_c.data_ptr(), lo_c.data_ptr(), hi_c.data_ptr(),
                     pids_c.data_ptr(), dead_c.data_ptr(), int(n_samples), int(seed) & 0xFFFFFFFF, out.data_ptr(),
                     _stream(dev))
    return out if ok else None


def _beta_wt(be) -> torch.Tensor:
    wt = getattr(be, "_beta_wt", None)
    if wt is None:
        import numpy as np

        with _LAZY_LOCK:
            wt = getattr(be, "_beta_wt", None)
            if wt is None:
                parts = []
                for w, b in zip(be.mlp.weights, be.mlp.biases):
                    parts += [np.ascontiguousarray(np.asarray(w, np.float32).T).reshape(-1),
                              np.zeros(np.size(b), np.float32)]
                wt = torch.from_numpy(np.concatenate(parts)).to(be.device)
                if wt.is_cuda:
                    torch.cuda.current_stream(wt.device).synchronize()
                be._beta_wt = wt
    return wt


def beta_batched_fits(be) -> bool:
    return bool(ext().beta_batched_fits(_net(be)))


def _beta_rows(be, lo, hi, pa, va, vb, LBA, UBA, LBB, UBB, phA, phB, rx, osg):
    R, n0 = lo.shape
    NH = be.n_hidden
    npa = len(pa)
    t = dict(flat=be.flat, lo=_c(lo, torch.float32, (R, n0), "lo"), hi=_c(hi, torch.float32, (R, n0), "hi"),
             va=_c(va, torch.float32, (R, npa), "va"), vb=_c(vb, torch.float32, (R, npa), "vb"))
    for x, nm in ((LBA, "LBA"), (UBA, "UBA"), (LBB, "LBB"), (UBB, "UBB")):
        t[nm] = _c(x, torch.float32, (R, NH), nm)
    t.update(phA=_c(phA, torch.int8, (R, NH), "phA"), phB=_c(phB, torch.int8, (R, NH), "phB"), plo=None, phi=None,
             gtie=None, osg=None if osg is None else _c(osg, torch.int8, (R,), "osg"))
    ramask, tau = 0, 0.0
    if rx is not None:
        for d in torch.nonzero(rx[0].cpu()).flatten().tolist():
            ramask |= 1 << int(d)
        t["plo"] = _c(rx[1], torch.float32, (R, n0), "plo")
        t["phi"] = _c(rx[2], torch.float32, (R, n0), "phi")
        if len(rx) > 3 and rx[4] is not None:
            tau = float(rx[3])
            for x, nm in ((rx[4], "gP"), (rx[5], "gM")):
                if tuple(x.shape) != (R, n0) or x.dtype != torch.float32:
                    raise ValueError(f"{nm}: expected float32 [{R}, {n0}]")
            t["gtie"] = torch.stack([rx[4], rx[5]], 1).contiguous()
    kw = dict(_ptrs(**t), R=R, pa=[int(d) for d in pa], ramask=int(ramask), tau=tau, stream=_stream(lo.device))
    return kw, t


def _beta_steps(iters, lr_a, lr_b, lr_t, decay):
    return dict(iters=int(iters), lr_a=float(lr_a), lr_b=float(lr_b), lr_t=float(lr_t), decay=float(decay))


def beta_opt16(be, lo, hi, pa, va, vb, LBA, UBA, LBB, UBB, phA, phB, alA, alB, beA, beB, t, iters, lr_a, lr_b, lr_t,
               decay=1.0, beta_pos=True, rx=None, pgap=0, osg=None):
    R, n0 = lo.shape
    NH = be.n_hidden
    dev = lo.device
    if list(pa) != sorted(pa):
        raise ValueError("beta_opt16: PA dims must be increasing")
    if not beta_batched_fits(be):
        raise RuntimeError("fa_beta_opt16_kernel: network not supported by the batched beta optimiser")
    f32 = dict(dtype=torch.float32, device=dev)
    kw, keep = _beta_rows(be, lo, hi, pa, va, vb, LBA, UBA, LBB, UBB, phA, phB, rx, osg)
    for x, nm in ((alA, "alA"), (alB, "alB"), (beA, "beA"), (beB, "beB")):
        if tuple(x.shape) != (R, NH) or x.dtype != torch.float32:
            raise ValueError(f"{nm}: expected float32 [{R}, {NH}]")
    if tuple(t.shape) != (R,) or t.dtype != torch.float32:
        raise ValueError("t: expected float32 [R]")
    par = torch.stack([alA, alB, beA, beB], 1).contiguous()
    t_o = t.clone().contiguous()
    gt = keep["gtie"]
    pgsum = torch.zeros(R, 4, NH, **f32)
    pgn = torch.zeros(R, **f32)
    if R:
        scratch = torch.empty(max(int(ext().beta_opt16_scratch(_net(be), R)), 1), **f32)
        rc = ext().beta_opt16(_net(be), **kw, **_ptrs(par=par, t=t_o, scratch=scratch, pgsum=pgsum, pgn=pgn),
                              **_beta_steps(iters, lr_a, lr_b, lr_t, decay), beta_pos=int(bool(beta_pos)),
                              flags=(int(pgap) & 3) << 1)
        if rc != 0:
            raise RuntimeError(f"fa_beta_opt16_kernel launch failed ({rc})")
    return par, t_o, (None if gt is None else gt[:, 0]), (None if gt is None else gt[:, 1]), pgsum, pgn


def beta_flags(stall, pgap, feas: bool = False) -> int:
    pg = int(pgap)
    if not 0 <= pg <= 3:
        raise ValueError(f"beta: pgap (BetaConfig.pgap_weights) must be 0, 1, 2 or 3, got {pgap!r}")
    return int(bool(stall)) | ((pg & 3) << 1) | (8 if feas else 0)


def _feas_buffers(be, R, n0, NH, tie, batched, dev):
    f32 = dict(dtype=torch.float32, device=dev)
    nscr = R * 16 * NH
    fpar = fgt = None
    if batched:
        nscr = max(nscr, int(ext().beta_opt16_scratch(_net(be), R)))
        fpar = torch.zeros(R, 4, NH, **f32)
        fgt = torch.zeros(R, 2, n0, **f32) if tie else None
    return torch.empty(max(nscr, 1), **f32), fpar, fgt


def beta_feas(be, lo, hi, pa, va, vb, LBA, UBA, LBB, UBB, phA, phB, alA, alB, t, bound, iters, lr, batched: bool,
              decay=1.0, rx=None, osg=None, proposal=None, return_proposal=False):
    R, n0 = lo.shape
    NH = be.n_hidden
    dev = lo.device
    if list(pa) != sorted(pa):
        raise ValueError("beta_feas: PA dims must be increasing")
    two_phase = bool(batched) or proposal is not None
    if two_phase and not beta_batched_fits(be):
        raise RuntimeError("fa_beta_opt16_kernel: network not supported by the batched beta optimiser")
    kw, keep = _beta_rows(be, lo, hi, pa, va, vb, LBA, UBA, LBB, UBB, phA, phB, rx, osg)
    for x, nm in ((alA, "alA"), (alB, "alB")):
        if tuple(x.shape) != (R, NH) or x.dtype != torch.float32:
            raise ValueError(f"{nm}: expected float32 [{R}, {NH}]")
    z = torch.zeros_like(alA)
    par = torch.stack([alA, alB, z, z], 1).contiguous()
    t_c = _c(t, torch.float32, (R,), "t").clone()
    bnd_o = _c(bound, torch.float64, (R,), "bound").clone()
    gt = keep["gtie"]
    fval = torch.full((R,), float("nan"), dtype=torch.float64, device=dev)
    scratch, fpar, fgt = _feas_buffers(be, R, n0, NH, gt is not None, two_phase, dev)
    mode = 1 if batched else 0
    if proposal is not None:
        mode = 3
        fpar = _c(proposal[0], torch.float32, (R, 4, NH), "fpar").clone()
        if gt is not None:
            fgt = _c(proposal[1], torch.float32, (R, 2, n0), "fgt").clone()
    if R:
        rc = ext().beta_feas(_net(be), **kw, **_beta_steps(iters, lr[0], lr[1], lr[2], decay), mode=mode,
                             **_ptrs(wt=_beta_wt(be), par=par, t=t_c, scratch=scratch, bound=bnd_o, fpar=fpar, fgt=fgt,
                                     fval=fval))
        if rc != 0:
            raise RuntimeError(f"beta_feas launch failed ({rc})")
    closed = torch.isinf(bnd_o) & (bnd_o > 0) & ~(torch.isinf(bound) & (bound > 0))
    if return_proposal:
        return closed, fval, (fpar, fgt)
    return closed, fval


def beta_level(be, lo, hi, pa, va, vb, LBA, UBA, LBB, UBB, phA, phB, alA, alB, beA, beB, t, iters, lr_a, lr_b, lr_t,
               decay=1.0, lookahead=0, beta_pos=True, rx=None, stall=True, pgap=False, osg=None, feas_iters=0,
               feas_lr=None, batched=False, batched_feas=False):
    from . import beta as B

    flags = beta_flags(stall, pgap)
    batched_feas = bool(batched and batched_feas and feas_iters > 0)

    R, n0 = lo.shape
    NH = be.n_hidden
    dev = lo.device
    if list(pa) != sorted(pa):
        raise ValueError("beta_level: PA dims must be increasing")
    f32 = dict(dtype=torch.float32, device=dev)
    kw, keep = _beta_rows(be, lo, hi, pa, va, vb, LBA, UBA, LBB, UBB, phA, phB, rx, osg)
    gt = keep["gtie"]
    for x, nm in ((alA, "alA"), (alB, "alB"), (beA, "beA"), (beB, "beB")):
        if tuple(x.shape) != (R, NH) or x.dtype != torch.float32:
            raise ValueError(f"{nm}: expected float32 [{R}, {NH}]")
    if tuple(t.shape) != (R,) or t.dtype != torch.float32 or not t.is_contiguous():
        raise ValueError("t: expected contiguous float32 [R]")
    par = torch.stack([alA, alB, beA, beB], 1).contiguous()
    nscr = R * (16 if feas_iters > 0 else 12) * NH
    pgsum = pgn = None
    if batched:
        if not beta_batched_fits(be):
            raise RuntimeError("fa_beta_opt16_kernel: network not supported by the batched beta optimiser")
        nscr = max(nscr, int(ext().beta_opt16_scratch(_net(be), R)))
        pgsum = torch.empty(R, 4, NH, **f32)
        pgn = torch.empty(R, **f32)
    scratch = torch.empty(max(nscr, 1), **f32)
    fpar = fgt = None
    if batched_feas:
        fpar = torch.empty(R, 4, NH, **f32)
    bound = torch.empty(R, dtype=torch.float64, device=dev)
    split = torch.empty(R, dtype=torch.int32, device=dev)
    xstar = torch.empty(R, n0, **f32)
    binit = torch.empty(R, 2, **f32)
    xpstar = torch.empty(R, n0, **f32)
    if batched_feas and gt is not None:
        fgt = torch.empty(R, 2, n0, **f32)
    if R:
        net = _net(be)
        kw.update(_ptrs(wt=_beta_wt(be), par=par, t=t, scratch=scratch, bound=bound, split=split, xstar=xstar,
                        binit=binit, xpstar=xpstar),
                  **_beta_steps(iters, lr_a, lr_b, lr_t, decay), lookahead=int(lookahead),
                  beta_pos=int(bool(beta_pos)), flags=flags)
        if batched:
            rc = ext().beta_level16(net, **kw, **_ptrs(pgsum=pgsum, pgn=pgn))
        else:
            rc = ext().beta_level(net, **kw)
        if rc == 0 and feas_iters > 0:
            fkw = {**kw, **_beta_steps(feas_iters, *(feas_lr or (lr_a, lr_b, lr_t)), decay)}
            if batched_feas:
                rc = ext().beta_feas(net, **fkw, **_ptrs(fpar=fpar, fgt=fgt), mode=1)
            else:
                rc = ext().beta_level(net, **{**fkw, "flags": beta_flags(False, 0, feas=True)})
        if rc != 0:
            raise RuntimeError(f"fa_beta_kernel launch failed ({rc}): network not supported by the beta kernel")
        if gt is not None:
            rx[4].copy_(gt[:, 0])
            rx[5].copy_(gt[:, 1])
        alA.copy_(par[:, 0])
        alB.copy_(par[:, 1])
        beA.copy_(par[:, 2])
        beB.copy_(par[:, 3])
    return B.BetaLevel(bound=bound, split=split.long(), xstar=xstar, binit=binit, xpstar=xpstar)
```

Before: 277,900.

## Add shaped symbolic-bound path with box prefetch, status skip, and PA value expansion

Extends the symbolic bounds kernel with a shape-specialised row loop. It prefetches the next row's box bounds per lane, expands protected-attribute values on the device, and skips rows whose partition status is already settled. The shaped path also uses compile-time LDS offsets, can leave out dead-mask reads and writes, and writes the final coefficient rows across all lanes, with a per-shape thread and waves-per-EU tuning table. A geometry query binding is added, and the Python side gains V/pa/values/skip options. These paths only run when callers pass the new arguments or the shape matches, and they add code complexity and a risk of correctness bugs.

Result: faster. 295,900, median of 6 (+6.5%).

```diff
diff --git a/fairify_amd/csrc/bindings.cpp b/fairify_amd/csrc/bindings.cpp
--- a/fairify_amd/csrc/bindings.cpp
+++ b/fairify_amd/csrc/bindings.cpp
@@ -20,6 +20,7 @@
 extern "C" int fa_sim_launch(const NetDesc& net, SimArgs a, hipStream_t stream);
 extern "C" int fa_sim_shaped(const NetDesc& net);
 extern "C" int fa_sym_shaped(const NetDesc& net, unsigned long long fold_mask);
+extern "C" int fa_sym_geometry(const NetDesc& net, unsigned long long fold_mask, int* out);
 extern "C" int fa_crown_shaped(const NetDesc& net, int mask);
 extern "C" int fa_refine_shaped(const NetDesc& net, int logit);
 extern "C" int fa_rate_launch(const NetDesc& net, RateArgs a, hipStream_t stream);
@@ -273,6 +274,14 @@
     a.fold = k.u64("fold", 0);
     a.phase_in = k.ptr<const int8_t>("phase_in");
     a.infeas = k.ptr<uint8_t>("infeas");
+    a.V = k.i("V", 0);
+    if (a.V > 0) {
+      a.npa = dims(k, "pa", a.pa_idx, FA_MAX_PA, "bounds: too many protected attributes");
+      a.values = k.need<const float>("values");
+    }
+    a.skip_status = k.ptr<const int8_t>("skip_status");
+    a.skip_part = k.ptr<const int>("skip_part");
+    if (a.skip_status && !a.skip_part) throw std::invalid_argument("bounds: skip_status without skip_part");
     ckl(fa_bounds_launch(net.d, a, finish(k)), "bounds");
   });
 
@@ -361,6 +370,20 @@
   });
   m.def("sim_shaped", [](const Net& net) { return fa_sim_shaped(net.d) != 0; });
   m.def("sym_shaped", [](const Net& net, unsigned long long fold) { return fa_sym_shaped(net.d, fold) != 0; });
+  m.def("sym_geometry", [](const Net& net, unsigned long long fold) -> py::object {
+    int g[8] = {0};
+    if (fa_sym_geometry(net.d, fold, g) != 1) return py::none();
+    py::dict d;
+    d["threads"] = g[0];
+    d["lds_bytes"] = g[1];
+    d["blocks_per_cu"] = g[2];
+    d["cus"] = g[3];
+    d["rows_per_block"] = g[4];
+    d["waves_per_simd"] = g[5];
+    d["shaped"] = g[6] != 0;
+    d["regs"] = g[7];
+    return d;
+  });
   m.def("crown_shaped", [](const Net& net, bool mask) { return fa_crown_shaped(net.d, mask) != 0; });
   m.def("refine_shaped", [](const Net& net, bool logit) { return fa_refine_shaped(net.d, logit) != 0; });
 
diff --git a/fairify_amd/csrc/symbolic.hip b/fairify_amd/csrc/symbolic.hip
--- a/fairify_amd/csrc/symbolic.hip
+++ b/fairify_amd/csrc/symbolic.hip
@@ -22,6 +22,28 @@
 template <int... D>
 using SymShape = FaShape<D...>;
 
+template <class S>
+struct SymLay {
+  __host__ __device__ static constexpr int tiles(int n) { return (n + 15) >> 4; }
+  __host__ __device__ static constexpr int w(int l) {
+    int off = 0;
+    for (int i = 0; i < l; ++i) off += tiles(S::dim(i)) * tiles(S::dim(i + 1)) * 256;
+    return off;
+  }
+  __host__ __device__ static constexpr int b(int l) {
+    int off = w(S::L);
+    for (int i = 0; i < l; ++i) off += S::dim(i + 1);
+    return off;
+  }
+  __host__ __device__ static constexpr int noff(int l) {
+    int off = 0;
+    for (int i = 0; i < l; ++i) off += S::dim(i + 1);
+    return off;
+  }
+  static constexpr int STAGE = (b(S::L) + 3) & ~3;
+  static constexpr int LDS = STAGE + FA_SYM_MAXC;
+};
+
 struct SymBox {
   const BoundArgs* a;
   int node, v, n0;
@@ -69,7 +91,7 @@
   }
 }
 
-template <int NT, bool PAIR, int PG = 1, bool CR = false, class S = SymShapeAny>
+template <int NT, bool PAIR, int PG = 1, bool CR = false, class S = SymShapeAny, bool MASK = true>
 __device__ __forceinline__ bool fa_sym_epilogue(const NetDesc& net, const BoundArgs& a, const SymCfg& cfg,
                                                 const float* smem, float* T, const float* bxv_in, const int* cdim_s,
                                                 int l, int r_in, int node_in, int r2, int node2, bool v2, int lane,
@@ -78,16 +100,17 @@
                                                 float (&nlo)[2][NT][4]) {
   constexpr int TS = SymSlab<NT>::TS;
   constexpr bool CS = S::L > 0;
+  constexpr bool CL = CS && PG == 1;
   const int col = lane & 15, grp = lane >> 4;
   const int n_out = CS ? S::dim(l + 1) : net.dims[l + 1];
-  const float* sb = smem + cfg.b_lds[l];
+  const float* sb = smem + (CL ? SymLay<S>::b(l) : cfg.b_lds[l]);
   const bool last = CS ? l == S::L - 1 : l == net.n_layers - 1;
   const float gg = net.g_gemm[l];
   const float gc = net.g_conc;
   const float gi = net.g_one;
   const float unit = net.unit;
   const float gnext = last ? 0.f : (CR ? net.g_fwd[l + 1] : net.g_gemm[l + 1]);
-  const int noff = net.neuron_off[l];
+  const int noff = CL ? SymLay<S>::noff(l) : net.neuron_off[l];
   const int nc = cfg.nc;
   const int n0 = CS ? S::dim(0) : net.dims[0];
   const int tsub = lane >> 5;
@@ -152,21 +175,40 @@
       else a.layer_lb[(size_t)r * net.n_neurons + noff + j] = lb;
     }
     if (last) {
-      if (nl_act && j == 0) {
-        float* Cf = ob == 0 ? a.Uc : a.Lc;
-        if (ob == 0) {
-          a.out_ub[r] = ub; a.U0[r] = c0; a.Ue[r] = e;
-        } else {
-          a.out_lb[r] = lb; a.L0[r] = c0; a.Le[r] = e;
-        }
-        for (int d = 0; d < n0; ++d)
-          if ((cfg.fold >> d) & 1ull) Cf[(size_t)r * n0 + d] = 0.f;
-        for (int c = 0; c < nc; ++c) Cf[(size_t)r * n0 + cdim_s[c]] = Trow[4 + c];
+      if (PG > 1) {
+        if (nl_act && j == 0) {
+          float* Cf = ob == 0 ? a.Uc : a.Lc;
+          if (ob == 0) {
+            a.out_ub[r] = ub; a.U0[r] = c0; a.Ue[r] = e;
+          } else {
+            a.out_lb[r] = lb; a.L0[r] = c0; a.Le[r] = e;
+          }
+          for (int d = 0; d < n0; ++d)
+            if ((cfg.fold >> d) & 1ull) Cf[(size_t)r * n0 + d] = 0.f;
+          for (int c = 0; c < nc; ++c) Cf[(size_t)r * n0 + cdim_s[c]] = Trow[4 + c];
+        }
+      } else if (nl_act && jt == 0) {
+        if (col == 0) {
+          if (ob == 0) {
+            a.out_ub[r] = ub; a.U0[r] = c0; a.Ue[r] = e;
+          } else {
+            a.out_lb[r] = lb; a.L0[r] = c0; a.Le[r] = e;
+          }
+        }
+        float* Cf = (ob == 0 ? a.Uc : a.Lc) + (size_t)r * n0;
+        const float* row0 = T + tsub * SymSlab<NT>::TILE1 + (ob * 16) * TS + fa_trot(ob * 16) + 4;
+        const unsigned long long fold = cfg.fold;
+        for (int d = col; d < n0; d += 16) {
+          const bool folded = (fold >> d) & 1ull;
+          const int c = d - __popcll(fold & ((1ull << d) - 1ull));
+          const float x = row0[folded ? 0 : c];
+          Cf[d] = folded ? 0.f : x;
+        }
       }
       return false;
     }
     bool forced = false, fact = false;
-    if (nl_act && jv) {
+    if (MASK && nl_act && jv) {
       if (a.dead_in) forced = a.dead_in[(size_t)r * net.n_hidden + noff + j] != 0;
       else if (a.dead_part) forced = a.dead_part[(size_t)a.node_part[node] * net.n_hidden + noff + j] != 0;
       if (a.phase_in) {
@@ -178,7 +220,7 @@
     }
     const bool isdead = ub <= 0.f;
     const bool isact = lb >= 0.f;
-    if (nl_act && ob == 0 && jv && a.dead_out) a.dead_out[(size_t)r * net.n_hidden + noff + j] = isdead ? 1 : 0;
+    if (MASK && nl_act && ob == 0 && jv && a.dead_out) a.dead_out[(size_t)r * net.n_hidden + noff + j] = isdead ? 1 : 0;
     const bool zero = isdead || forced || !jv;
     const float aa = mn - gc * mg + e;
     const float bb = mx + gc * mg + e;
@@ -228,7 +270,7 @@
     return true;
 }
 
-template <int NT, int TM, bool PAIR, int PG = 1, class S = SymShapeAny>
+template <int NT, int TM, bool PAIR, int PG = 1, class S = SymShapeAny, bool MASK = true>
 __device__ __forceinline__ void fa_sym_layer(const NetDesc& net, const BoundArgs& a, const SymCfg& cfg,
                                              const float* smem, float* T, const float* bxv, const int* cdim_s,
                                              int l, int r, int node, int r2, int node2, bool v2, int lane,
@@ -238,22 +280,15 @@
   constexpr bool CR = SymForm<PAIR, TM>::CR;
   constexpr int TS = SymSlab<NT>::TS;
   constexpr bool CS = S::L > 0;
+  constexpr bool CL = CS && PG == 1;
   const int col = lane & 15, grp = lane >> 4;
   const int n_in = CS ? S::dim(l) : net.dims[l], n_out = CS ? S::dim(l + 1) : net.dims[l + 1];
   const int tin = (n_in + 15) >> 4, tout = (n_out + 15) >> 4;
-  const float* sw = smem + cfg.w_lds[l];
-  const float* sb = smem + cfg.b_lds[l];
+  const float* sw = smem + (CL ? SymLay<S>::w(l) : cfg.w_lds[l]);
   const bool last = CS ? l == S::L - 1 : l == net.n_layers - 1;
   const float gg = net.g_gemm[l];
-  const float gc = net.g_conc;
-  const float gi = net.g_one;
-  const float unit = net.unit;
-  const float gnext = last ? 0.f : net.g_gemm[l + 1];
-  const int noff = net.neuron_off[l];
   const int nc = cfg.nc;
   const int n0 = CS ? S::dim(0) : net.dims[0];
-  const bool nl_act = lane < 32;
-  const int ob = (lane >> 4) & 1;
 #ifndef FA_SYM_TIMING_NO_EPILOGUE
   if (PG > 1 && l == 0) {
     const float* boxtab = bxv + 2 * PG * SymSlab<NT, PG>::BOX;
@@ -303,7 +338,7 @@
       }
     }
     float nu[2][NT][4], nlo[2][NT][4];
-    if (!fa_sym_epilogue<NT, PAIR, PG, CR, S>(net, a, cfg, smem, T, bxv, cdim_s, l, r, node, r2, node2, v2, lane, 0, U, Lq,
+    if (!fa_sym_epilogue<NT, PAIR, PG, CR, S, MASK>(net, a, cfg, smem, T, bxv, cdim_s, l, r, node, r2, node2, v2, lane, 0, U, Lq,
                                        nu, nlo))
       return;
 #pragma unroll
@@ -364,7 +399,7 @@
         if (CR) fa_pq_to_ul(f32x4(U[bi][ct]), f32x4(Lq[bi][ct]), ct * 16 + col, gg, U[bi][ct], Lq[bi][ct]);
       }
     float nu[2][NT][4], nlo[2][NT][4];
-    fa_sym_epilogue<NT, PAIR, PG, CR, S>(net, a, cfg, smem, T, bxv, cdim_s, l, r, node, r2, node2, v2, lane, 0, U, Lq,
+    fa_sym_epilogue<NT, PAIR, PG, CR, S, MASK>(net, a, cfg, smem, T, bxv, cdim_s, l, r, node, r2, node2, v2, lane, 0, U, Lq,
                                   nu, nlo);
     return;
   }
@@ -429,7 +464,7 @@
       continue;
     }
 #else
-    if (!fa_sym_epilogue<NT, PAIR, PG, CR, S>(net, a, cfg, smem, T, bxv, cdim_s, l, r, node, r2, node2, v2, lane, jt0, U,
+    if (!fa_sym_epilogue<NT, PAIR, PG, CR, S, MASK>(net, a, cfg, smem, T, bxv, cdim_s, l, r, node, r2, node2, v2, lane, jt0, U,
                                        Lq, nu, nlo))
       continue;
 #endif
@@ -456,16 +491,16 @@
 #define FA_SYM_WAVES_PER_EU(NT, TM, PAIR) \
   ((PAIR) ? 3 : ((TM) == 2 ? 3 : ((TM) == 4 ? FA_SYM_WPE4 : ((TM) == 7 ? FA_SYM_WPE7 : 1))))
 
-template <int NT, int TM, bool PAIR, int PG, class S, int... LS>
+template <int NT, int TM, bool PAIR, int PG, class S, bool MASK, int... LS>
 __device__ __forceinline__ void fa_sym_layers_c(std::integer_sequence<int, LS...>, const NetDesc& net,
                                                 const BoundArgs& a, const SymCfg& cfg, const float* smem, float* T,
                                                 const float* bxv, const int* cdim_s, int r, int node, int r2,
                                                 int node2, bool v2, int lane, float (&XA)[NT][PAIR ? 2 : TM][2][4],
                                                 float (&XB)[NT][PAIR ? 2 : TM][2][4]) {
-  ((LS & 1 ? fa_sym_layer<NT, TM, PAIR, PG, S>(net, a, cfg, smem, T, bxv, cdim_s, LS, r, node, r2, node2, v2, lane,
-                                               XB, XA)
-           : fa_sym_layer<NT, TM, PAIR, PG, S>(net, a, cfg, smem, T, bxv, cdim_s, LS, r, node, r2, node2, v2, lane,
-                                               XA, XB)),
+  ((LS & 1 ? fa_sym_layer<NT, TM, PAIR, PG, S, MASK>(net, a, cfg, smem, T, bxv, cdim_s, LS, r, node, r2, node2, v2,
+                                                     lane, XB, XA)
+           : fa_sym_layer<NT, TM, PAIR, PG, S, MASK>(net, a, cfg, smem, T, bxv, cdim_s, LS, r, node, r2, node2, v2,
+                                                     lane, XA, XB)),
    ...);
 }
 
@@ -474,29 +509,79 @@
 #endif
 #define FA_SYM_THREADS(TM) ((TM) == 7 ? FA_SYM_BIG_THREADS : FA_THREADS)
 
-template <int NT, int TM, bool PAIR, int PG = 1, class S = SymShapeAny>
-__global__ void __launch_bounds__(FA_SYM_THREADS(TM)) __attribute__((amdgpu_waves_per_eu(FA_SYM_WAVES_PER_EU(NT, TM, PAIR))))
-fa_sym_kernel(NetDesc net, BoundArgs a, SymCfg cfg) {
+#ifndef FA_SYM_PREFETCH
+#define FA_SYM_PREFETCH 1
+#endif
+
+template <int NT, int TM, bool PAIR, class S>
+struct SymTune {
+  static constexpr int THREADS = FA_SYM_THREADS(TM);
+  static constexpr int WPE = FA_SYM_WAVES_PER_EU(NT, TM, PAIR);
+};
+#define FA_SYM_TUNE(NT, TM, THREADS_, WPE_, ...)            \
+  template <>                                                \
+  struct SymTune<NT, TM, false, FaShape<__VA_ARGS__>> {      \
+    static constexpr int THREADS = THREADS_;                 \
+    static constexpr int WPE = WPE_;                         \
+  };
+FA_SYM_TUNE(1, 7, 256, 3, 13, 100, 1)
+
+__device__ __forceinline__ void fa_sym_box_values(float l0, float h0, float* bv, int lane) {
+  float mid = 0.5f * (l0 + h0), rad = 0.5f * (h0 - l0), mm = fmaxf(fabsf(l0), fabsf(h0));
+  const bool lattice = l0 == rintf(l0) && h0 == rintf(h0) && fabsf(l0) < 4194304.f && fabsf(h0) < 4194304.f;
+  if (!lattice) {
+    rad = nextafterf(fmaxf(h0 - mid, mid - l0), INFINITY);
+    mm = nextafterf(fabsf(mid) + rad, INFINITY);
+  }
+  bv[lane] = mid;
+  bv[FA_SYM_MAXC + lane] = rad;
+  bv[2 * FA_SYM_MAXC + lane] = mm;
+}
+
+template <int NT, bool CR, int TMS>
+__device__ __forceinline__ void fa_sym_operand0(float xl, float xh, bool kv, bool folded, int k, float g0,
+                                                const int (&role)[NT], const int (&cdm)[NT],
+                                                float (&XA)[NT][TMS][2][4], int t, int i) {
+  const float m = fmaxf(fabsf(xl), fabsf(xh));
+#pragma unroll
+  for (int ct = 0; ct < NT; ++ct) {
+    float vu = 0.f, vl = 0.f;
+    if (kv) {
+      switch (role[ct]) {
+        case 0: vu = (!folded && cdm[ct] == k) ? 1.f : 0.f; vl = CR ? 0.f : vu; break;
+        case 1: vu = folded ? xl : 0.f; vl = CR ? 0.f : vu; break;
+        case 2: vu = CR ? 0.f : g0 * m; vl = CR ? g0 * m : -vu; break;
+        case 3:
+          vu = CR ? 0.5f * (xh + xl) : xh;
+          vl = CR ? 0.5f * (xh - xl) : xl;
+          break;
+        case 4:
+          vu = CR ? 0.5f * g0 * (fabsf(xh) - fabsf(xl)) : g0 * fabsf(xh);
+          vl = CR ? 0.5f * g0 * (fabsf(xh) + fabsf(xl)) : -(g0 * fabsf(xl));
+          break;
+        default: break;
+      }
+    }
+    XA[ct][t][0][i] = vu;
+    XA[ct][t][1][i] = vl;
+  }
+}
+
+template <int NT, int TM, bool PAIR, int PG, class S, bool MASK>
+__device__ __forceinline__ void fa_sym_rows(const NetDesc& net, const BoundArgs& a, const SymCfg& cfg, float* smem,
+                                            const int* cdim_s, int lds_floats) {
+  constexpr int THREADS = SymTune<NT, TM, PAIR, S>::THREADS;
   constexpr bool CR = SymForm<PAIR, TM>::CR;
   constexpr int TMS = PAIR ? 2 : TM;
-  extern __shared__ __attribute__((aligned(16))) float smem[];
   const int tid = threadIdx.x;
-  {
-    const float4* src = reinterpret_cast<const float4*>(a.flat + cfg.stage_off);
-    float4* dst = reinterpret_cast<float4*>(smem);
-    for (int e = tid; e < (cfg.stage_floats >> 2); e += FA_SYM_THREADS(TM)) dst[e] = src[e];
-  }
-  int* cdim_s = reinterpret_cast<int*>(smem + cfg.lds_floats - FA_SYM_MAXC);
-  for (int c = tid; c < FA_SYM_MAXC; c += FA_SYM_THREADS(TM)) cdim_s[c] = c < cfg.nc ? cfg.cdim[c] : -1;
-  __syncthreads();
   const int lane = tid & 63;
   const int grp = lane >> 4;
   const int wave = tid >> 6;
-  const int nw = FA_SYM_THREADS(TM) / 64;
+  const int nw = THREADS / 64;
   const int n0 = S::L > 0 ? S::dim(0) : net.dims[0];
   const int nc = cfg.nc;
   const float g0 = net.g_gemm[0];
-  float* T = smem + cfg.lds_floats + wave * SymSlab<NT, PG>::FLOATS;
+  float* T = smem + lds_floats + wave * SymSlab<NT, PG>::FLOATS;
   float* bxv = T + SymSlab<NT>::TILE;
   const int tin0 = (n0 + 15) >> 4;
   int role[NT], cdm[NT];
@@ -507,6 +592,80 @@
     cdm[ct] = (role[ct] == 0) ? cdim_s[c - 4] : -1;
   }
   constexpr int RPW = PAIR ? 2 * PG : 1;
+  if constexpr (!PAIR && S::L > 0 && FA_SYM_PREFETCH) {
+    float* btab = bxv + SymSlab<NT>::BOX;
+    static_assert(SymSlab<NT>::BOX >= 128, "box table in the second box's slot");
+    static_assert(S::dim(0) <= 64, "lane d carries input dim d");
+    const int V = a.V, R = a.R;
+    int pslot = -1;
+    if (V > 0)
+      for (int k = 0; k < a.npa; ++k)
+        if (a.pa_idx[k] == lane) pslot = k;
+    const int dl = min(lane, n0 - 1);
+    const int stride = gridDim.x * nw;
+    const bool filt = a.skip_status != nullptr;
+    auto node_of = [&](int rr) { return V > 0 ? rr / V : rr; };
+    auto fetch = [&](int rr, int node, float& blo, float& bhi) {
+      blo = a.lo[(size_t)node * n0 + dl];
+      bhi = a.hi[(size_t)node * n0 + dl];
+      if (pslot >= 0) blo = bhi = a.values[(rr - node * V) * a.npa + pslot];
+    };
+    int r = __builtin_amdgcn_readfirstlane(blockIdx.x * nw + wave);
+    float blo = 0.f, bhi = 0.f;
+    int st = 3, part1 = 0;
+    int node = 0;
+    if (r < R) {
+      node = node_of(r);
+      fetch(r, node, blo, bhi);
+      if (filt) st = a.skip_status[a.skip_part[node]];
+      if (filt && r + stride < R) part1 = a.skip_part[node_of(r + stride)];
+    }
+    for (; r < R; r += stride) {
+      const int rn = r + stride;
+      float nlo = 0.f, nhi = 0.f;
+      int nst = 3, part2 = 0, nnode = 0;
+      if (rn < R) {
+        nnode = node_of(rn);
+        fetch(rn, nnode, nlo, nhi);
+        if (filt) nst = a.skip_status[part1];
+        if (filt && rn + stride < R) part2 = a.skip_part[node_of(rn + stride)];
+      }
+      if (st == 3 || st == 4) {
+        btab[lane] = blo;
+        btab[64 + lane] = bhi;
+        __builtin_amdgcn_wave_barrier();
+        if (lane < FA_SYM_MAXC) {
+          const int d = (lane >= 4 && lane - 4 < nc) ? cdim_s[lane - 4] : -1;
+          fa_sym_box_values(d >= 0 ? btab[max(d, 0)] : 0.f, d >= 0 ? btab[64 + max(d, 0)] : 0.f, bxv, lane);
+        }
+        float XA[NT][TMS][2][4], XB[NT][TMS][2][4];
+#pragma unroll
+        for (int t = 0; t < TMS; ++t) {
+          if (t >= tin0) break;
+          const float4 l4 = reinterpret_cast<const float4*>(btab)[(4 * t + grp) & 15];
+          const float4 h4 = reinterpret_cast<const float4*>(btab + 64)[(4 * t + grp) & 15];
+          const float xl4[4] = {l4.x, l4.y, l4.z, l4.w}, xh4[4] = {h4.x, h4.y, h4.z, h4.w};
+#pragma unroll
+          for (int i = 0; i < 4; ++i) {
+            const int k = 16 * t + 4 * grp + i;
+            const bool kv = k < n0;
+            const float xl = kv ? xl4[i] : 0.f, xh = kv ? xh4[i] : 0.f;
+            fa_sym_operand0<NT, CR>(xl, xh, kv, kv && ((cfg.fold >> k) & 1ull), k, g0, role, cdm, XA, t, i);
+          }
+        }
+        __builtin_amdgcn_wave_barrier();
+        fa_sym_layers_c<NT, TM, PAIR, PG, S, MASK>(std::make_integer_sequence<int, S::L>{}, net, a, cfg, smem, T, bxv,
+                                                   cdim_s, r, node, r, node, false, lane, XA, XB);
+        __builtin_amdgcn_wave_barrier();
+      }
+      blo = nlo;
+      bhi = nhi;
+      st = nst;
+      part1 = part2;
+      node = nnode;
+    }
+    return;
+  }
   for (int r0 = (blockIdx.x * nw + wave) * RPW; r0 < a.R; r0 += gridDim.x * nw * RPW) {
     const int r = __builtin_amdgcn_readfirstlane(r0);
     const bool v2 = PAIR && r + 1 < a.R;
@@ -533,16 +692,7 @@
       if (lane < FA_SYM_MAXC) {
         float* bv = bxv + bi * SymSlab<NT>::BOX;
         const int d = (lane >= 4 && lane - 4 < nc) ? cdim_s[lane - 4] : -1;
-        const float l0 = d >= 0 ? bx.lo(d) : 0.f, h0 = d >= 0 ? bx.hi(d) : 0.f;
-        float mid = 0.5f * (l0 + h0), rad = 0.5f * (h0 - l0), mm = fmaxf(fabsf(l0), fabsf(h0));
-        const bool lattice = l0 == rintf(l0) && h0 == rintf(h0) && fabsf(l0) < 4194304.f && fabsf(h0) < 4194304.f;
-        if (!lattice) {
-          rad = nextafterf(fmaxf(h0 - mid, mid - l0), INFINITY);
-          mm = nextafterf(fabsf(mid) + rad, INFINITY);
-        }
-        bv[lane] = mid;
-        bv[FA_SYM_MAXC + lane] = rad;
-        bv[2 * FA_SYM_MAXC + lane] = mm;
+        fa_sym_box_values(d >= 0 ? bx.lo(d) : 0.f, d >= 0 ? bx.hi(d) : 0.f, bv, lane);
       }
       if (PG > 1 && lane < 32) {
         const int d = lane & 15;
@@ -566,48 +716,48 @@
           xl = bt.lo(k);
           xh = bt.hi(k);
         }
-        const bool folded = kv && ((cfg.fold >> k) & 1ull);
-        const float m = fmaxf(fabsf(xl), fabsf(xh));
-#pragma unroll
-        for (int ct = 0; ct < NT; ++ct) {
-          float vu = 0.f, vl = 0.f;
-          if (kv) {
-            switch (role[ct]) {
-              case 0: vu = (!folded && cdm[ct] == k) ? 1.f : 0.f; vl = CR ? 0.f : vu; break;
-              case 1: vu = folded ? xl : 0.f; vl = CR ? 0.f : vu; break;
-              case 2: vu = CR ? 0.f : g0 * m; vl = CR ? g0 * m : -vu; break;
-              case 3:
-                vu = CR ? 0.5f * (xh + xl) : xh;
-                vl = CR ? 0.5f * (xh - xl) : xl;
-                break;
-              case 4:
-                vu = CR ? 0.5f * g0 * (fabsf(xh) - fabsf(xl)) : g0 * fabsf(xh);
-                vl = CR ? 0.5f * g0 * (fabsf(xh) + fabsf(xl)) : -(g0 * fabsf(xl));
-                break;
-              default: break;
-            }
-          }
-          XA[ct][t][0][i] = vu;
-          XA[ct][t][1][i] = vl;
-        }
+        fa_sym_operand0<NT, CR>(xl, xh, kv, kv && ((cfg.fold >> k) & 1ull), k, g0, role, cdm, XA, t, i);
       }
     }
     __builtin_amdgcn_wave_barrier();
     if constexpr (S::L > 0) {
-      fa_sym_layers_c<NT, TM, PAIR, PG, S>(std::make_integer_sequence<int, S::L>{}, net, a, cfg, smem, T, bxv, cdim_s,
-                                           r, bx.node, rb, bxs[RPW - 1].node, v2, lane, XA, XB);
+      fa_sym_layers_c<NT, TM, PAIR, PG, S, MASK>(std::make_integer_sequence<int, S::L>{}, net, a, cfg, smem, T, bxv,
+                                                 cdim_s, r, bx.node, rb, bxs[RPW - 1].node, v2, lane, XA, XB);
     } else {
       for (int l = 0; l < net.n_layers; ++l) {
         if (l & 1)
-          fa_sym_layer<NT, TM, PAIR, PG>(net, a, cfg, smem, T, bxv, cdim_s, l, r, bx.node, rb, bxs[RPW - 1].node, v2,
-                                         lane, XB, XA);
+          fa_sym_layer<NT, TM, PAIR, PG, S, MASK>(net, a, cfg, smem, T, bxv, cdim_s, l, r, bx.node, rb,
+                                                  bxs[RPW - 1].node, v2, lane, XB, XA);
         else
-          fa_sym_layer<NT, TM, PAIR, PG>(net, a, cfg, smem, T, bxv, cdim_s, l, r, bx.node, rb, bxs[RPW - 1].node, v2,
-                                         lane, XA, XB);
+          fa_sym_layer<NT, TM, PAIR, PG, S, MASK>(net, a, cfg, smem, T, bxv, cdim_s, l, r, bx.node, rb,
+                                                  bxs[RPW - 1].node, v2, lane, XA, XB);
       }
     }
     __builtin_amdgcn_wave_barrier();
   }
+}
+
+template <int NT, int TM, bool PAIR, int PG = 1, class S = SymShapeAny>
+__global__ void __launch_bounds__((SymTune<NT, TM, PAIR, S>::THREADS))
+    __attribute__((amdgpu_waves_per_eu(SymTune<NT, TM, PAIR, S>::WPE))) fa_sym_kernel(NetDesc net, BoundArgs a, SymCfg cfg) {
+  constexpr int THREADS = SymTune<NT, TM, PAIR, S>::THREADS;
+  constexpr bool CL = S::L > 0 && PG == 1;
+  extern __shared__ __attribute__((aligned(16))) float smem[];
+  const int tid = threadIdx.x;
+  const int stage_floats = CL ? SymLay<S>::STAGE : cfg.stage_floats;
+  const int lds_floats = CL ? SymLay<S>::LDS : cfg.lds_floats;
+  {
+    const float4* src = reinterpret_cast<const float4*>(a.flat + cfg.stage_off);
+    float4* dst = reinterpret_cast<float4*>(smem);
+    for (int e = tid; e < (stage_floats >> 2); e += THREADS) dst[e] = src[e];
+  }
+  int* cdim_s = reinterpret_cast<int*>(smem + lds_floats - FA_SYM_MAXC);
+  for (int c = tid; c < FA_SYM_MAXC; c += THREADS) cdim_s[c] = c < cfg.nc ? cfg.cdim[c] : -1;
+  __syncthreads();
+  constexpr bool LEAN = S::L > 0 && !PAIR;
+  const bool masked = !LEAN || a.dead_in || a.dead_part || a.phase_in || a.dead_out;
+  if (masked) fa_sym_rows<NT, TM, PAIR, PG, S, true>(net, a, cfg, smem, cdim_s, lds_floats);
+  else fa_sym_rows<NT, TM, PAIR, PG, S, !LEAN>(net, a, cfg, smem, cdim_s, lds_floats);
 }
 
 
@@ -691,12 +841,37 @@
 
 constexpr int sym_key(int nt, int tm, bool pair, int pg) { return ((16 * nt + tm) * 2 + (pair ? 1 : 0)) * 8 + pg; }
 
+typedef bool (*SymLayoutOk)(const NetDesc&, const SymCfg&);
+struct SymInst {
+  SymKernel k = nullptr;
+  SymLayoutOk ok = nullptr;
+  int threads = 0, wpe = 0;
+  SymInst(std::nullptr_t = nullptr) {}
+  SymInst(SymKernel k_, SymLayoutOk ok_, int threads_, int wpe_) : k(k_), ok(ok_), threads(threads_), wpe(wpe_) {}
+};
+template <class S>
+bool sym_layout_ok(const NetDesc& net, const SymCfg& cfg);
+template <int NT, int TM, bool PAIR, int PG, class S>
+SymInst sym_inst() {
+  typedef SymTune<NT, TM, PAIR, S> Tune;
+  return SymInst(fa_sym_kernel<NT, TM, PAIR, PG, S>, sym_layout_ok<S>, Tune::THREADS, Tune::WPE);
+}
+template <class S>
+bool sym_layout_ok(const NetDesc& net, const SymCfg& cfg) {
+  for (int l = 0; l < S::L; ++l)
+    if (cfg.w_lds[l] != SymLay<S>::w(l) || cfg.b_lds[l] != SymLay<S>::b(l) || net.neuron_off[l] != SymLay<S>::noff(l))
+      return false;
+  return cfg.stage_floats == SymLay<S>::STAGE && cfg.lds_floats == SymLay<S>::LDS;
+}
+
 struct SymPick {
   SymKernel k;
   int NT, tmb;
   bool pair;
   int pg;
   bool shaped;
+  int threads, wpe;
+  int err;
 };
 
 SymPick pick_sym(const NetDesc& net, unsigned long long fold_mask, SymCfg& cfg) {
@@ -711,6 +886,10 @@
       cfg.cdim[nc++] = d;
     }
   cfg.nc = nc;
+  if (n0 < 64 && (fold_mask >> n0)) return p;
+  if (nc != n0 - __builtin_popcountll(fold_mask)) return p;
+  for (int c = 1; c < nc; ++c)
+    if (cfg.cdim[c] <= cfg.cdim[c - 1]) return p;
   const int cols = nc + 4;
   p.NT = (cols + 15) / 16;
   p.tmb = tm_bucket(p.NT, fa_widest_tiles(net, 0, net.n_layers));
@@ -720,18 +899,68 @@
   p.pg = (p.pair && net.pack_g > 1 && net.dims[0] <= 16 && use_pack()) ? net.pack_g : 1;
   if (p.pg > 1) k = select_packed(p.pg);
   if (!k) return p;
+  int off = 0;
+  if (p.pg > 1) {
+    cfg.w_lds[0] = 0;
+    off = p.pg * 256;
+    for (int l = 1; l < net.n_layers; ++l) {
+      cfg.w_lds[l] = off;
+      off += 256;
+    }
+    for (int l = 0; l < net.n_layers; ++l) {
+      cfg.b_lds[l] = off;
+      off += 16;
+    }
+    if (off != net.pack_floats) p.err = -1;
+    cfg.stage_off = net.pack_off;
+  } else {
+    off = fa_lay_weights(net, net.n_layers, cfg.w_lds, 0);
+    off = fa_lay_biases(net, net.n_layers, cfg.b_lds, off);
+    off = ((off + 3) & ~3);
+    if (off != net.wperm_floats) p.err = -1;
+    cfg.stage_off = net.wperm_off;
+  }
+  cfg.stage_floats = off;
+  cfg.lds_floats = off + FA_SYM_MAXC;
+  p.threads = FA_SYM_THREADS(p.pair ? 1 : p.tmb);
+  p.wpe = FA_SYM_WAVES_PER_EU(p.NT, p.tmb, p.pair);
   if (!fa_env_off("FAIRIFY_SYM_SHAPED")) {
 #define FA_SYM_ENTRY(NT, TM, PAIR, PG, ...) \
-  {sym_key(NT, TM, PAIR, PG), {__VA_ARGS__}, fa_sym_kernel<NT, TM, PAIR, PG, SymShape<__VA_ARGS__>>},
-    static const std::vector<FaShaped<SymKernel>> v = {FA_SYM_SHAPES(FA_SYM_ENTRY)};
+  {sym_key(NT, TM, PAIR, PG),                \
+   {__VA_ARGS__},                            \
+   sym_inst<NT, TM, PAIR, PG, SymShape<__VA_ARGS__>>()},
+    static const std::vector<FaShaped<SymInst>> v = {FA_SYM_SHAPES(FA_SYM_ENTRY)};
 #undef FA_SYM_ENTRY
-    if (const SymKernel ks = fa_find_shaped(v, net, sym_key(p.NT, p.tmb, p.pair, p.pg))) {
-      k = ks;
+    const SymInst si = fa_find_shaped(v, net, sym_key(p.NT, p.tmb, p.pair, p.pg));
+    if (si.k && !p.err && (p.pg > 1 || si.ok(net, cfg))) {
+      k = si.k;
       p.shaped = true;
+      p.threads = si.threads;
+      p.wpe = si.wpe;
     }
   }
   p.k = k;
   return p;
+}
+
+struct SymGeom {
+  int threads, rows_per_block;
+  size_t bytes;
+};
+SymGeom sym_geom(const SymPick& p, const SymCfg& cfg) {
+  int slab = 0;
+  switch (p.NT) {
+    case 1:
+      slab = p.pg == 2 ? SymSlab<1, 2>::FLOATS : p.pg == 4 ? SymSlab<1, 4>::FLOATS : SymSlab<1>::FLOATS;
+      break;
+    case 2: slab = SymSlab<2>::FLOATS; break;
+    default: slab = SymSlab<3>::FLOATS; break;
+  }
+  SymGeom g;
+  g.threads = p.threads;
+  g.rows_per_block = (g.threads / 64) * (p.pair ? 2 * p.pg : 1);
+  g.bytes = (size_t)(cfg.lds_floats + (g.threads / 64) * slab) * sizeof(float);
+  return g;
 }
 
 }
@@ -748,52 +977,37 @@
   const SymPick p = pick_sym(net, fold_mask, cfg);
   const SymKernel k = p.k;
   if (!k) return 0;
-  const int NT = p.NT, tmb = p.tmb, pg = p.pg;
-  const bool pair0 = p.pair;
-  int off = 0;
-  if (pg > 1) {
-    cfg.w_lds[0] = 0;
-    off = pg * 256;
-    for (int l = 1; l < net.n_layers; ++l) {
-      cfg.w_lds[l] = off;
-      off += 256;
-    }
-    for (int l = 0; l < net.n_layers; ++l) {
-      cfg.b_lds[l] = off;
-      off += 16;
-    }
-    if (off != net.pack_floats) return -1;
-    cfg.stage_off = net.pack_off;
-  } else {
-    off = fa_lay_weights(net, net.n_layers, cfg.w_lds, 0);
-    off = fa_lay_biases(net, net.n_layers, cfg.b_lds, off);
-    off = ((off + 3) & ~3);
-    if (off != net.wperm_floats) return -1;
-    cfg.stage_off = net.wperm_off;
-  }
-  cfg.stage_floats = off;
-  off += FA_SYM_MAXC;
-  cfg.lds_floats = off;
-  int slab = 0;
-  switch (NT) {
-    case 1:
-      slab = pg == 2 ? SymSlab<1, 2>::FLOATS : pg == 4 ? SymSlab<1, 4>::FLOATS : SymSlab<1>::FLOATS;
-      break;
-    case 2: slab = SymSlab<2>::FLOATS; break;
-    default: slab = SymSlab<3>::FLOATS; break;
-  }
-  const int threads = (!pair0 && NT == 1 && tmb == 7) ? FA_SYM_BIG_THREADS : FA_THREADS;
-  const int rows_per_block = (threads / 64) * (pair0 ? 2 * pg : 1);
-  const size_t bytes = (size_t)(off + (threads / 64) * slab) * sizeof(float);
-  if (bytes > 160 * 1024) return 0;
-  const int per_cu = fa_blocks_per_cu((const void*)k, threads, bytes);
+  if (p.err) return p.err;
+  const SymGeom g = sym_geom(p, cfg);
+  if (g.bytes > 160 * 1024) return 0;
+  const int per_cu = fa_blocks_per_cu((const void*)k, g.threads, g.bytes);
   if (!per_cu) return -4;
-  long long blocks = (a.R + rows_per_block - 1) / rows_per_block;
+  long long blocks = (a.R + g.rows_per_block - 1) / g.rows_per_block;
   const long long cap = (long long)fa_device_cus() * per_cu;
   if (blocks > cap) blocks = cap;
-  hipLaunchKernelGGL(k, dim3((unsigned)blocks), dim3(threads), bytes, stream, net, a, cfg);
+  hipLaunchKernelGGL(k, dim3((unsigned)blocks), dim3(g.threads), g.bytes, stream, net, a, cfg);
   const hipError_t e = hipGetLastError();
   return e == hipSuccess ? 1 : -(int)e;
+}
+
+extern "C" int fa_sym_geometry(const NetDesc& net, unsigned long long fold_mask, int* out) {
+  SymCfg cfg{};
+  const SymPick p = pick_sym(net, fold_mask, cfg);
+  if (!p.k || p.err) return 0;
+  const SymGeom g = sym_geom(p, cfg);
+  if (g.bytes > 160 * 1024) return 0;
+  const int per_cu = fa_blocks_per_cu((const void*)p.k, g.threads, g.bytes);
+  if (!per_cu) return 0;
+  out[0] = g.threads;
+  out[1] = (int)g.bytes;
+  out[2] = per_cu;
+  out[3] = fa_device_cus();
+  out[4] = g.rows_per_block;
+  out[5] = p.wpe;
+  out[6] = p.shaped;
+  hipFuncAttributes fa{};
+  out[7] = hipFuncGetAttributes(&fa, (const void*)p.k) == hipSuccess ? fa.numRegs : 0;
+  return 1;
 }
 
 #define FA_SYM_LDS(NT, TM) FA_LDS_K((sym_ptr<NT, TM>())),
diff --git a/fairify_amd/ops/hip.py b/fairify_amd/ops/hip.py
--- a/fairify_amd/ops/hip.py
+++ b/fairify_amd/ops/hip.py
@@ -56,9 +56,10 @@
     return {k: t.data_ptr() for k, t in tensors.items() if t is not None}
 
 
-def _bound_kw(be, lo, hi, dead=None, res=None, layer_lb=None, layer_ub=None):
-    R, n0 = lo.shape
-    t = dict(flat=be.flat, lo=_c(lo, torch.float32, (R, n0), "lo"), hi=_c(hi, torch.float32, (R, n0), "hi"),
+def _bound_kw(be, lo, hi, dead=None, res=None, layer_lb=None, layer_ub=None, rows=None):
+    B, n0 = lo.shape
+    R = B if rows is None else rows
+    t = dict(flat=be.flat, lo=_c(lo, torch.float32, (B, n0), "lo"), hi=_c(hi, torch.float32, (B, n0), "hi"),
              dead_in=None if dead is None else _c(dead, torch.uint8, (R, be.n_hidden), "dead"),
              layer_lb=layer_lb, layer_ub=layer_ub)
     if res is not None:
@@ -176,35 +177,59 @@
 
 def bounds(be, lo: torch.Tensor, hi: torch.Tensor, mode: str = "symbolic", dead: Optional[torch.Tensor] = None,
            keep_layers: bool = False, G: int = 0, fold: Sequence[int] = (),
-           phase: Optional[torch.Tensor] = None) -> ref.BoundResult:
+           phase: Optional[torch.Tensor] = None, *, dead_out: bool = True, V: int = 0, pa: Sequence[int] = (),
+           values: Optional[torch.Tensor] = None, skip_status: Optional[torch.Tensor] = None,
+           skip_part: Optional[torch.Tensor] = None, fill: Optional[float] = None) -> ref.BoundResult:
     R, n0 = lo.shape
     if n0 != be.n0:
         raise ValueError(f"box width {n0} != network input {be.n0}")
+    if V < 0 or (V > 0 and (values is None or not len(pa))):
+        raise ValueError("bounds: V > 0 needs pa and values [V, len(pa)]")
+    if (skip_status is None) != (skip_part is None):
+        raise ValueError("bounds: skip_status and skip_part go together")
+    if V > 0:
+        R *= V
     dev = lo.device
     sym = 1 if mode == "symbolic" else 0
     f32 = dict(dtype=torch.float32, device=dev)
-    res = ref.BoundResult(out_lb=torch.empty(R, **f32), out_ub=torch.empty(R, **f32))
+
+    def new(*shape, dtype=torch.float32):
+        if fill is None:
+            return torch.empty(*shape, dtype=dtype, device=dev)
+        return torch.full(shape, fill if dtype.is_floating_point else 0xEE, dtype=dtype, device=dev)
+
+    res = ref.BoundResult(out_lb=new(R), out_ub=new(R))
     if sym:
-        res.Lc = torch.empty(R, n0, **f32)
-        res.L0 = torch.empty(R, **f32)
-        res.Le = torch.empty(R, **f32)
-        res.Uc = torch.empty(R, n0, **f32)
-        res.U0 = torch.empty(R, **f32)
-        res.Ue = torch.empty(R, **f32)
+        res.Lc = new(R, n0)
+        res.L0 = new(R)
+        res.Le = new(R)
+        res.Uc = new(R, n0)
+        res.U0 = new(R)
+        res.Ue = new(R)
     N = be.mlp.n_neurons
     lay_lb = lay_ub = None
     if keep_layers:
-        lay_lb = torch.empty(R, N, **f32)
-        lay_ub = torch.empty(R, N, **f32)
-    dead_out = torch.empty(R, be.n_hidden, dtype=torch.uint8, device=dev) if be.n_hidden else None
+        lay_lb = new(R, N)
+        lay_ub = new(R, N)
+    dead_out = new(R, be.n_hidden, dtype=torch.uint8) if be.n_hidden and dead_out else None
     ph = infeas = None
     if phase is not None:
         ph = _c(phase, torch.int8, (R, be.n_hidden), "phase")
         infeas = torch.zeros(R, dtype=torch.uint8, device=dev)
-    kw, _keep = _bound_kw(be, lo, hi, dead, res, lay_lb, lay_ub)
+    kw, _keep = _bound_kw(be, lo, hi, dead, res, lay_lb, lay_ub, rows=R)
+    bab = {}
+    if V > 0:
+        vals = _c(values, torch.float32, (V, len(pa)), "values")
+        bab.update(V=V, pa=[int(d) for d in pa], values=vals.data_ptr())
+    if skip_status is not None:
+        st = _c(skip_status, torch.int8, None, "skip_status")
+        sp = _c(skip_part, torch.int32, (lo.shape[0],), "skip_part")
+        if st.dim() != 1 or (sp.numel() and (int(sp.min()) < 0 or int(sp.max()) >= st.shape[0])):
+            raise ValueError("bounds: skip_part indexes outside skip_status")
+        bab.update(skip_status=st.data_ptr(), skip_part=sp.data_ptr())
     if R:
         ext().bounds(_net(be), **kw, **_ptrs(dead_out=dead_out, phase_in=ph, infeas=infeas), symbolic=sym, G=G,
-                     fold=_fold_mask(fold, n0))
+                     fold=_fold_mask(fold, n0), **bab)
     if infeas is not None:
         res.infeasible = infeas.bool()
     if keep_layers:
```
